# FoundationVision/OmniTokenizer

Measured on NVIDIA H100. Metric: video_frames_per_sec_encode_decode, higher is better.
Workload: dtype f32

## Files before the change

### include/omnitok_b200.h

```cpp
#ifndef OMNITOK_B200_H_
#define OMNITOK_B200_H_

#include <stdint.h>

#ifdef __cplusplus
extern "C" {
#endif

#define OMT_ABI_VERSION 2

#define OMT_OK 0
#define OMT_E_ARG (-1)
#define OMT_E_ARCH (-2)
#define OMT_E_CUDA (-3)
#define OMT_E_UNSUPPORTED (-4)

typedef void* omt_stream_t;

int omt_abi_version(void);
const char* omt_last_error(void);
int omt_device_info(int* sm_count, int* cc_major, int* cc_minor);

#define OMT_EPI_NONE 0
#define OMT_EPI_GEGLU 1
#define OMT_EPI_QKV 2
#define OMT_EPI_QKV_PLANES 3

#define OMT_MATH_FP32 0
#define OMT_MATH_3XTF32 1
#define OMT_MATH_F16X3 3

int omt_linear(const float* A, int lda, int a_seg, int a_seg_stride, int a_seg_off,
               const float* W, const float* W_lo,
               float* C, int ldc, int c_seg, int c_seg_stride, int c_seg_off,
               int M, int N, int K,
               const float* bias, const float* residual, int ldr,
               int epilogue, int math, omt_stream_t stream);

int omt_linear2(const float* A1, const float* A2, int n_split, int lda, const float* W, const float* W_lo,
                float* C, int ldc, int M, int N, int K, int math,
                const float* q_scale, const float* k_scale, const float* rope_cos, const float* rope_sin,
                int qk_cols, int tokens, omt_stream_t stream);

int omt_layernorm(const float* x, int ldx, float* y, int ldy, const float* w, const float* b,
                  int M, int C, float eps, int seg, int seg_stride, int seg_off, omt_stream_t stream);

int omt_patchify_ln(const float* video, float* A, uint16_t* A_hi, uint16_t* A_lo, float* A_rs, const float* ln_w, const float* ln_b,
                    int B, int Cin, int T, int H, int W, int p, int pt, int first, float eps,
                    omt_stream_t stream);

int omt_patchify_ln_u8(const uint8_t* frames, const float* lut, const int32_t* sel, float* A, uint16_t* A_hi, uint16_t* A_lo,
                       float* A_rs, const float* ln_w, const float* ln_b, int B, int Cin, int T, int H, int W, int p, int pt,
                       int first, float eps, omt_stream_t stream);

int omt_u8_norm_select(const uint8_t* frames, int B, long long per_sample, int32_t* sel, omt_stream_t stream);

int omt_unpatchify(const float* P, float* video, int B, int Cin, int T, int H, int W, int p, int pt,
                   int first, omt_stream_t stream);

int omt_unpatchify_u8(const float* P, uint8_t* out, int B, int Cin, int T, int H, int W, int p, int pt,
                      int first, float mul, float add, float lo, float hi, float post, omt_stream_t stream);

int omt_peg(const float* x, float* y, const float* w27, const float* bias, const int32_t* nbr,
            int B, int rows_per_b, int C, omt_stream_t stream);

int omt_peg_volume(const float* x, float* y, const float* w27, const float* bias, int B, int T, int h, int w,
                   int C, int temporal, int causal, omt_stream_t stream);

int omt_qk_prep(float* q, int ldq, float* k, int ldk, const float* q_scale, const float* k_scale,
                const float* rope_cos, const float* rope_sin, int M, int N, int heads,
                omt_stream_t stream);

int omt_attn_spatial(const float* q, int ldq, const float* k, int ldk, const float* v, int ldv,
                     float* o, uint16_t* o_hi, uint16_t* o_lo, int ldo, int n_seq, int N, int heads, float scale,
                     omt_stream_t stream);

int omt_attn_spatial_h(const uint16_t* q_hi, const uint16_t* q_lo, int ldq, const uint16_t* k_hi, const uint16_t* k_lo, int ldk,
                       const uint16_t* v_hi, const uint16_t* v_lo, int ldv, const float* vinv, float qk_plane_scale,
                       float* o, uint16_t* o_hi, uint16_t* o_lo, int ldo, int n_seq, int N, int heads, float scale,
                       omt_stream_t stream);

int omt_attn_window(const float* q, int ldq, const float* k, int ldk, const float* v, int ldv,
                    float* o, uint16_t* o_hi, uint16_t* o_lo, int ldo, const float* bias, int n_frames, int h, int w, int ws, int heads,
                    float scale, omt_stream_t stream);

int omt_attn_temporal(const float* q, int ldq, const float* k, int ldk, const float* v, int ldv,
                      float* o, uint16_t* o_hi, uint16_t* o_lo, int ldo, int B, int T, int N, int heads, float scale, int causal,
                      omt_stream_t stream);

int omt_pre_vq(const float* x, int ldx, const float* Wt, const float* b, float* z, int M, int C, int cd,
               int l2, omt_stream_t stream);

int omt_vq_search(const float* z, const float* E, const float* e2, int M, int n_codes,
                  int64_t* idx, int32_t* counts, omt_stream_t stream);

int omt_vq_fused(const float* x, int ldx, const float* Wt, const float* b, int C, int l2, float* z,
                 const float* E, const float* e2, int M, int n_codes, int64_t* idx, int32_t* counts,
                 omt_stream_t stream);

int omt_post_vq(const int64_t* idx, const float* E, const float* zc, const float* z_st_from,
                float* zq_out, const float* Wt, const float* b, float* X, int M, int C, int cd,
                omt_stream_t stream);

typedef struct omt_linear_h_args {
  const uint16_t* a_hi; const uint16_t* a_lo;
  const float* a_rs; const float* a2_rs;
  float w_scale;
  const uint16_t* a2_hi; const uint16_t* a2_lo;
  int n_split;
  int lda, a_seg, a_seg_stride, a_seg_off;
  const uint16_t* w_hi; const uint16_t* w_lo;
  float* c; int ldc, c_seg, c_seg_stride, c_seg_off;
  uint16_t* u_hi; uint16_t* u_lo; int ldu;
  int M, N, K;
  const float* bias; const float* residual; int ldr;
  int epilogue;
  const float* q_scale; const float* k_scale; const float* rope_cos; const float* rope_sin;
  int qk_cols, tokens;
  float q_plane_scale, k_plane_scale;
  float* vinv;
  float a_rs_uniform, u_scale;
} omt_linear_h_args;

int omt_linear_h(const omt_linear_h_args* args, omt_stream_t stream);

int omt_layernorm_h(const float* x, int ldx, float* y, int ldy, uint16_t* y_hi, uint16_t* y_lo, float* y_rs,
                    uint16_t* x_hi, uint16_t* x_lo, float* x_rs, int lds, const float* w, const float* b,
                    int M, int C, float eps, int seg, int seg_stride, int seg_off, omt_stream_t stream);

int omt_set_option(const char* name, int value);

#ifdef __cplusplus
}
#endif
#endif
```

### omnitokenizer_b200/_cabi.py

```python
from __future__ import annotations

import ctypes
import os
from ctypes import c_char_p, c_float, c_int, c_int64, c_void_p, POINTER

import torch

_LIB_NAME = "libomnitok_b200.so"
_lib = None

EPI_NONE, EPI_GEGLU, EPI_QKV, EPI_QKV_PLANES = 0, 1, 2, 3
MATH_FP32, MATH_3XTF32, MATH_F16X3 = 0, 1, 3
ABI_VERSION = 2


class LinearHArgs(ctypes.Structure):
    _fields_ = [("a_hi", c_void_p), ("a_lo", c_void_p), ("a_rs", c_void_p), ("a2_rs", c_void_p), ("w_scale", c_float),
                ("a2_hi", c_void_p), ("a2_lo", c_void_p), ("n_split", c_int),
                ("lda", c_int), ("a_seg", c_int), ("a_seg_stride", c_int), ("a_seg_off", c_int),
                ("w_hi", c_void_p), ("w_lo", c_void_p),
                ("c", c_void_p), ("ldc", c_int), ("c_seg", c_int), ("c_seg_stride", c_int), ("c_seg_off", c_int),
                ("u_hi", c_void_p), ("u_lo", c_void_p), ("ldu", c_int),
                ("M", c_int), ("N", c_int), ("K", c_int),
                ("bias", c_void_p), ("residual", c_void_p), ("ldr", c_int),
                ("epilogue", c_int),
                ("q_scale", c_void_p), ("k_scale", c_void_p), ("rope_cos", c_void_p), ("rope_sin", c_void_p),
                ("qk_cols", c_int), ("tokens", c_int),
                ("q_plane_scale", c_float), ("k_plane_scale", c_float), ("vinv", c_void_p),
                ("a_rs_uniform", c_float), ("u_scale", c_float)]


SIGNATURES = {
    "omt_abi_version": (c_int, []),
    "omt_last_error": (c_char_p, []),
    "omt_device_info": (c_int, [POINTER(c_int)] * 3),
    "omt_set_option": (c_int, [c_char_p, c_int]),
    "omt_linear": (c_int, [c_void_p, c_int, c_int, c_int, c_int, c_void_p, c_void_p, c_void_p, c_int, c_int, c_int,
                           c_int, c_int, c_int, c_int, c_void_p, c_void_p, c_int, c_int, c_int, c_void_p]),
    "omt_linear2": (c_int, [c_void_p, c_void_p, c_int, c_int, c_void_p, c_void_p, c_void_p, c_int, c_int, c_int, c_int,
                            c_int, c_void_p, c_void_p, c_void_p, c_void_p, c_int, c_int, c_void_p]),
    "omt_linear_h": (c_int, [POINTER(LinearHArgs), c_void_p]),
    "omt_layernorm": (c_int, [c_void_p, c_int, c_void_p, c_int, c_void_p, c_void_p, c_int, c_int, c_float, c_int, c_int,
                              c_int, c_void_p]),
    "omt_layernorm_h": (c_int, [c_void_p, c_int, c_void_p, c_int, c_void_p, c_void_p, c_void_p, c_void_p, c_void_p, c_void_p,
                                c_int, c_void_p, c_void_p, c_int, c_int, c_float, c_int, c_int, c_int, c_void_p]),
    "omt_patchify_ln": (c_int, [c_void_p, c_void_p, c_void_p, c_void_p, c_void_p, c_void_p, c_void_p] + [c_int] * 8 + [c_float, c_void_p]),
    "omt_patchify_ln_u8": (c_int, [c_void_p] * 9 + [c_int] * 8 + [c_float, c_void_p]),
    "omt_u8_norm_select": (c_int, [c_void_p, c_int, c_int64, c_void_p, c_void_p]),
    "omt_unpatchify": (c_int, [c_void_p, c_void_p] + [c_int] * 8 + [c_void_p]),
    "omt_unpatchify_u8": (c_int, [c_void_p, c_void_p] + [c_int] * 8 + [c_float] * 5 + [c_void_p]),
    "omt_peg": (c_int, [c_void_p, c_void_p, c_void_p, c_void_p, c_void_p, c_int, c_int, c_int, c_void_p]),
    "omt_peg_volume": (c_int, [c_void_p, c_void_p, c_void_p, c_void_p] + [c_int] * 7 + [c_void_p]),
    "omt_qk_prep": (c_int, [c_void_p, c_int, c_void_p, c_int, c_void_p, c_void_p, c_void_p, c_void_p, c_int, c_int,
                            c_int, c_void_p]),
    "omt_attn_spatial": (c_int, [c_void_p, c_int, c_void_p, c_int, c_void_p, c_int, c_void_p, c_void_p, c_void_p, c_int,
                                 c_int, c_int, c_int, c_float, c_void_p]),
    "omt_attn_spatial_h": (c_int, [c_void_p, c_void_p, c_int, c_void_p, c_void_p, c_int, c_void_p, c_void_p, c_int, c_void_p,
                                   c_float, c_void_p, c_void_p, c_void_p, c_int, c_int, c_int, c_int, c_float, c_void_p]),
    "omt_attn_window": (c_int, [c_void_p, c_int, c_void_p, c_int, c_void_p, c_int, c_void_p, c_void_p, c_void_p, c_int,
                                c_void_p, c_int, c_int, c_int, c_int, c_int, c_float, c_void_p]),
    "omt_attn_temporal": (c_int, [c_void_p, c_int, c_void_p, c_int, c_void_p, c_int, c_void_p, c_void_p, c_void_p, c_int,
                                  c_int, c_int, c_int, c_int, c_float, c_int, c_void_p]),
    "omt_pre_vq": (c_int, [c_void_p, c_int, c_void_p, c_void_p, c_void_p, c_int, c_int, c_int, c_int, c_void_p]),
    "omt_vq_search": (c_int, [c_void_p, c_void_p, c_void_p, c_int, c_int, c_void_p, c_void_p, c_void_p]),
    "omt_vq_fused": (c_int, [c_void_p, c_int, c_void_p, c_void_p, c_int, c_int, c_void_p, c_void_p, c_void_p, c_int, c_int,
                             c_void_p, c_void_p, c_void_p]),
    "omt_post_vq": (c_int, [c_void_p] * 8 + [c_int, c_int, c_int, c_void_p]),
}


def lib_path() -> str:
    return os.environ.get("OMT_LIB") or os.path.join(os.path.dirname(os.path.abspath(__file__)), _LIB_NAME)


def load():
    global _lib
    if _lib is not None:
        return _lib
    path = lib_path()
    if not os.path.exists(path):
        raise RuntimeError(
            f"{path} not found: the CUDA extension is not built. Run `python -c 'import __graft_entry__ as g; "
            f"g.build()'` (or `make -C omnitokenizer_b200/csrc`). There is no CPU fallback.")
    lib = ctypes.CDLL(path)
    for name, (res, args) in SIGNATURES.items():
        fn = getattr(lib, name)
        fn.restype = res
        fn.argtypes = args
    if lib.omt_abi_version() != ABI_VERSION:
        raise RuntimeError("libomnitok_b200.so ABI version mismatch")
    _lib = lib
    return lib


def _ptr(t):
    if t is None:
        return None
    if isinstance(t, int):
        return t
    return t.data_ptr()


def _stream():
    return torch.cuda.current_stream().cuda_stream


KERNELS_PER_CALL = {"omt_u8_norm_select": 2}
launch_count = 0


def call(name: str, *args):
    global launch_count
    lib = load()
    launch_count += KERNELS_PER_CALL.get(name, 1)
    conv = [_ptr(a) if (a is None or isinstance(a, torch.Tensor)) else a for a in args]
    rc = getattr(lib, name)(*conv, _stream())
    if rc != 0:
        raise RuntimeError(f"{name} failed ({rc}): {lib.omt_last_error().decode()}")


def linear_h(**kw):
    global launch_count
    lib = load()
    a = LinearHArgs()
    for k, v in kw.items():
        setattr(a, k, _ptr(v) if (v is None or isinstance(v, torch.Tensor)) else v)
    launch_count += 1
    rc = lib.omt_linear_h(ctypes.byref(a), _stream())
    if rc != 0:
        raise RuntimeError(f"omt_linear_h failed ({rc}): {lib.omt_last_error().decode()}")


DEFAULT_OPTIONS = {"attn_kernel": 3, "peg_kernel": 4, "f16_bn": 0, "attn_f16_ctas": 2}


def set_option(name: str, value: int):
    lib = load()
    rc = lib.omt_set_option(name.encode(), int(value))
    if rc != 0:
        raise RuntimeError(f"omt_set_option({name}) failed: {lib.omt_last_error().decode()}")


def device_info():
    lib = load()
    a, b, c = c_int(), c_int(), c_int()
    rc = lib.omt_device_info(ctypes.byref(a), ctypes.byref(b), ctypes.byref(c))
    if rc != 0:
        raise RuntimeError(lib.omt_last_error().decode())
    return a.value, b.value, c.value
```

### omnitokenizer_b200/csrc/attention_f16.cu

```cuda
#include "omt_common.cuh"
#include "tc_ptx.cuh"
#include <cuda.h>

namespace omt {
int g_attn_f16_ctas = 2;
namespace af16 {
using namespace omt::ptx;

constexpr int QT = 128, KT = 64, D = 64;
constexpr int TILE = KT * D * 2;
constexpr int STAGES = 4;
constexpr int OFF_Q = 0;
constexpr int OFF_KV = 4 * TILE;
constexpr int OFF_VI = OFF_KV + STAGES * 4 * TILE;
constexpr int OFF_CTRL = OFF_VI + STAGES * KT * 4;
constexpr int SMEM = OFF_CTRL + 128 + 1024;
constexpr int THREADS = 384;
constexpr uint32_t KV_BYTES = 4 * TILE + KT * 4;
constexpr int PRODUCER_REGS = 40, CONSUMER_REGS = 232;

struct Args {
  const float* vinv;
  long long rows;
  float* o; uint16_t* o_hi; uint16_t* o_lo; int ldo;
  int N, heads, items;
  float scale_log2;
};

__global__ void __launch_bounds__(THREADS, 1)
attn_f16_kernel(const __grid_constant__ CUtensorMap tmQh, const __grid_constant__ CUtensorMap tmQl,
                const __grid_constant__ CUtensorMap tmKh, const __grid_constant__ CUtensorMap tmKl,
                const __grid_constant__ CUtensorMap tmVh, const __grid_constant__ CUtensorMap tmVl, const Args a) {
  extern __shared__ uint8_t smem_raw[];
  uint8_t* smem = smem_raw + ((1024u - (smem_u32(smem_raw) & 1023u)) & 1023u);
  uint64_t* bars = reinterpret_cast<uint64_t*>(smem + OFF_CTRL);
  uint64_t& q_full = bars[0];
  uint64_t& q_empty = bars[1];
  uint64_t* full = bars + 2;
  uint64_t* empty = full + STAGES;
  float* vmax = reinterpret_cast<float*>(bars + 2 + 2 * STAGES);

  const int tid = threadIdx.x, warp = tid >> 5, lane = tid & 31;
  const int ntiles = a.N / KT, nqt = a.N / QT;

  if (tid == 0) {
    prefetch_map(&tmQh); prefetch_map(&tmQl); prefetch_map(&tmKh); prefetch_map(&tmKl); prefetch_map(&tmVh); prefetch_map(&tmVl);
    mbar_init(&q_full, 1);
    mbar_init(&q_empty, 256);
    for (int s = 0; s < STAGES; ++s) { mbar_init(&full[s], 1); mbar_init(&empty[s], 2); }
    fence_barrier_init();
  }
  __syncthreads();
  pdl_sync();

  auto decode = [&](int item, int& row_q0, int& row_k0, int& col0, int& head) {
    const int qt = item % nqt, hs = item / nqt, seq = hs / a.heads;
    head = hs % a.heads;
    row_k0 = seq * a.N;
    row_q0 = row_k0 + qt * QT;
    col0 = head * D;
  };

  if (warp < 4) {
    setmaxnreg_dec<PRODUCER_REGS>();
    if (warp == 0) {
      uint32_t it = 0, c = 0;
      for (int item = blockIdx.x; item < a.items; item += gridDim.x, ++c) {
        int row_q0, row_k0, col0, head;
        decode(item, row_q0, row_k0, col0, head);
        const float* vinv_h = a.vinv + (size_t)head * a.rows + row_k0;
        float vmx = 0.f;
        for (int i = 4 * lane; i < a.N; i += 128) {
          const float4 v = __ldg(reinterpret_cast<const float4*>(vinv_h + i));
          vmx = fmaxf(vmx, fmaxf(fmaxf(v.x, v.y), fmaxf(v.z, v.w)));
        }
        vmx = warp_max(vmx);
        mbar_wait(&q_empty, (c & 1) ^ 1);
        if (lane == 0) {
          *vmax = vmx;
          mbar_expect_tx(&q_full, 4 * TILE);
          for (int w = 0; w < 2; ++w) {
            tma_load_2d(&tmQh, &q_full, smem + OFF_Q + w * TILE, col0, row_q0 + w * 64);
            tma_load_2d(&tmQl, &q_full, smem + OFF_Q + (2 + w) * TILE, col0, row_q0 + w * 64);
          }
        }
        for (int j = 0; j < ntiles; ++j, ++it) {
          const int s = it % STAGES;
          mbar_wait(&empty[s], ((it / STAGES) & 1) ^ 1);
          if (lane == 0) {
            uint8_t* sp = smem + OFF_KV + s * 4 * TILE;
            const int kr = row_k0 + j * KT;
            mbar_expect_tx(&full[s], KV_BYTES);
            tma_load_2d(&tmKh, &full[s], sp, col0, kr);
            tma_load_2d(&tmKl, &full[s], sp + TILE, col0, kr);
            tma_load_2d(&tmVh, &full[s], sp + 2 * TILE, col0, kr);
            tma_load_2d(&tmVl, &full[s], sp + 3 * TILE, col0, kr);
            bulk_load(smem + OFF_VI + s * KT * 4, vinv_h + j * KT, KT * 4, &full[s]);
          }
        }
      }
    }
  } else {
    setmaxnreg_inc<CONSUMER_REGS>();
    const int wg = (warp >> 2) - 1, qd = lane & 3;
    const int rl0 = (warp & 3) * 16 + (lane >> 2);
    const uint32_t sb = smem_u32(smem);
    auto release = [&](uint32_t t) {
      if ((tid & 127) == 0) mbar_arrive(&empty[t % STAGES]);
    };
    float sv[32];
#pragma unroll
    for (int i = 0; i < 32; ++i) sv[i] = 0.f;
    uint32_t it = 0, c = 0;
    for (int item = blockIdx.x; item < a.items; item += gridDim.x, ++c) {
      int row_q0, row_k0, col0, head;
      decode(item, row_q0, row_k0, col0, head);
      mbar_wait(&q_full, c & 1);
      float p_scale, p_inv;
      row_scale(*vmax, p_scale, p_inv);
      uint32_t qh[16], ql[16];
#pragma unroll
      for (int kk = 0; kk < 4; ++kk)
#pragma unroll
        for (int e = 0; e < 2; ++e)
#pragma unroll
          for (int h = 0; h < 2; ++h) {
            const int r = rl0 + 8 * h;
            const uint8_t* p = smem + OFF_Q + wg * TILE + r * 128 + (((2 * kk + e) ^ (r & 7)) << 4) + qd * 4;
            qh[4 * kk + 2 * e + h] = *reinterpret_cast<const uint32_t*>(p);
            ql[4 * kk + 2 * e + h] = *reinterpret_cast<const uint32_t*>(p + 2 * TILE);
          }
      mbar_arrive(&q_empty);

      float o_acc[32];
#pragma unroll
      for (int i = 0; i < 32; ++i) o_acc[i] = 0.f;
      float m_run[2] = {-INFINITY, -INFINITY}, l_run[2] = {0.f, 0.f};
      uint32_t p_a[2][16], p_b[2][16];
      float alpha[2];

      auto wait_full = [&](uint32_t t) { mbar_wait(&full[t % STAGES], (t / STAGES) & 1); };
      auto issue_s = [&](uint32_t t) {
        const uint32_t kv = sb + OFF_KV + (t % STAGES) * 4 * TILE;
        const uint64_t dk_hi = desc_sw128(kv), dk_lo = desc_sw128(kv + TILE);
#pragma unroll
        for (int kk = 0; kk < 4; ++kk) {
          const uint64_t adv = (uint64_t)(kk * 2);
          wgmma_f16_n64_ra<0>(sv, ql + 4 * kk, dk_hi + adv, kk != 0);
          wgmma_f16_n64_ra<0>(sv, qh + 4 * kk, dk_lo + adv, 1);
          wgmma_f16_n64_ra<0>(sv, qh + 4 * kk, dk_hi + adv, 1);
        }
      };
      auto issue_pv = [&](const uint32_t (&p)[2][16], uint32_t t) {
        const uint32_t vh = sb + OFF_KV + (t % STAGES) * 4 * TILE + 2 * TILE, vl = vh + TILE;
#pragma unroll
        for (int kk = 0; kk < 4; ++kk) {
          const uint64_t dvh = desc_sw128(vh + kk * 2048), dvl = desc_sw128(vl + kk * 2048);
          wgmma_f16_n64_ra<1>(o_acc, p[1] + 4 * kk, dvh, 1);
          wgmma_f16_n64_ra<1>(o_acc, p[0] + 4 * kk, dvl, 1);
          wgmma_f16_n64_ra<1>(o_acc, p[0] + 4 * kk, dvh, 1);
        }
      };
      auto softmax = [&](uint32_t (&p)[2][16], uint32_t t) {
        float nm[2];
#pragma unroll
        for (int h = 0; h < 2; ++h) {
          float mx = -INFINITY;
#pragma unroll
          for (int jj = 0; jj < 8; ++jj) mx = fmaxf(mx, fmaxf(sv[4 * jj + 2 * h], sv[4 * jj + 2 * h + 1]));
          mx = fmaxf(mx, __shfl_xor_sync(0xffffffffu, mx, 1));
          mx = fmaxf(mx, __shfl_xor_sync(0xffffffffu, mx, 2));
          const float m_new = fmaxf(m_run[h], mx);
          alpha[h] = ex2_fast((m_run[h] - m_new) * a.scale_log2);
          m_run[h] = m_new;
          nm[h] = -m_new;
        }
        const float* vi = reinterpret_cast<const float*>(smem + OFF_VI + (t % STAGES) * KT * 4);
        float ps[2] = {0.f, 0.f};
#pragma unroll
        for (int jj = 0; jj < 8; ++jj) {
          const float2 w = *reinterpret_cast<const float2*>(vi + 8 * jj + 2 * qd);
#pragma unroll
          for (int h = 0; h < 2; ++h) {
            const float e0 = ex2_fast((sv[4 * jj + 2 * h] + nm[h]) * a.scale_log2);
            const float e1 = ex2_fast((sv[4 * jj + 2 * h + 1] + nm[h]) * a.scale_log2);
            ps[h] += e0 + e1;
            const int wd = 4 * (jj >> 1) + 2 * (jj & 1) + h;
            split2u(e0 * (w.x * p_scale), e1 * (w.y * p_scale), p[0][wd], p[1][wd]);
          }
        }
#pragma unroll
        for (int h = 0; h < 2; ++h) l_run[h] = fmaf(l_run[h], alpha[h], ps[h]);
      };
      auto rescale = [&]() {
#pragma unroll
        for (int h = 0; h < 2; ++h)
#pragma unroll
          for (int jj = 0; jj < 8; ++jj) { o_acc[4 * jj + 2 * h] *= alpha[h]; o_acc[4 * jj + 2 * h + 1] *= alpha[h]; }
      };
      auto step = [&](const uint32_t (&p)[2][16], uint32_t (&pn)[2][16], int j, bool next) {
        const uint32_t t = it + j;
        if (next) wait_full(t + 1);
        reg_fence(sv);
        reg_fence(o_acc);
        wg_fence();
        if (next) {
          issue_s(t + 1);
          wg_commit();
        }
        issue_pv(p, t);
        wg_commit();
        if (next) {
          wg_wait<1>();
          reg_fence(sv);
          softmax(pn, t + 1);
        }
        wg_wait<0>();
        reg_fence(o_acc);
        release(t);
        if (next) rescale();
      };

      wait_full(it);
      reg_fence(sv);
      wg_fence();
      issue_s(it);
      wg_commit();
      wg_wait<0>();
      reg_fence(sv);
      softmax(p_a, it);
      rescale();
      int j = 0;
      for (; j + 2 < ntiles; j += 2) {
        step(p_a, p_b, j, true);
        step(p_b, p_a, j + 1, true);
      }
      step(p_a, p_b, j, true);
      step(p_b, p_a, j + 1, false);
      it += ntiles;

#pragma unroll
      for (int h = 0; h < 2; ++h) {
        float l = l_run[h];
        l += __shfl_xor_sync(0xffffffffu, l, 1);
        l += __shfl_xor_sync(0xffffffffu, l, 2);
        const float inv = p_inv / l;
        const size_t ooff = (size_t)(row_q0 + wg * 64 + rl0 + 8 * h) * a.ldo + col0 + 2 * qd;
#pragma unroll
        for (int jj = 0; jj < 8; ++jj) {
          const float2 ov = make_float2(o_acc[4 * jj + 2 * h] * inv, o_acc[4 * jj + 2 * h + 1] * inv);
          if (a.o_hi != nullptr) store_split2(a.o_hi, a.o_lo, ooff + 8 * jj, ov);
          else *reinterpret_cast<float2*>(a.o + ooff + 8 * jj) = ov;
        }
      }
    }
  }
}

typedef CUresult (*EncodeTiledFn)(CUtensorMap*, CUtensorMapDataType, cuuint32_t, void*, const cuuint64_t*,
                                  const cuuint64_t*, const cuuint32_t*, const cuuint32_t*, CUtensorMapInterleave,
                                  CUtensorMapSwizzle, CUtensorMapL2promotion, CUtensorMapFloatOOBfill);

static int encode2d(CUtensorMap* m, const uint16_t* base, int cols, long long rows, int ld) {
  static EncodeTiledFn fn = nullptr;
  if (fn == nullptr) {
    void* p = nullptr;
    cudaDriverEntryPointQueryResult qres;
    if (cudaGetDriverEntryPoint("cuTensorMapEncodeTiled", &p, cudaEnableDefault, &qres) == cudaSuccess &&
        qres == cudaDriverEntryPointSuccess)
      fn = reinterpret_cast<EncodeTiledFn>(p);
  }
  if (fn == nullptr) { set_error("cuTensorMapEncodeTiled entry point not found"); return OMT_E_CUDA; }
  cuuint64_t dims[2] = {(cuuint64_t)cols, (cuuint64_t)rows};
  cuuint64_t strides[1] = {(cuuint64_t)ld * 2};
  cuuint32_t box[2] = {64, (cuuint32_t)KT};
  cuuint32_t estr[2] = {1, 1};
  CUresult r = fn(m, CU_TENSOR_MAP_DATA_TYPE_FLOAT16, 2, const_cast<uint16_t*>(base), dims, strides, box, estr,
                  CU_TENSOR_MAP_INTERLEAVE_NONE, CU_TENSOR_MAP_SWIZZLE_128B, CU_TENSOR_MAP_L2_PROMOTION_L2_256B,
                  CU_TENSOR_MAP_FLOAT_OOB_FILL_NONE);
  if (r != CUDA_SUCCESS) { set_error("cuTensorMapEncodeTiled failed (%d)", (int)r); return OMT_E_CUDA; }
  return OMT_OK;
}

}
}

using namespace omt;

extern "C" int omt_attn_spatial_h(const uint16_t* q_hi, const uint16_t* q_lo, int ldq, const uint16_t* k_hi,
                                  const uint16_t* k_lo, int ldk, const uint16_t* v_hi, const uint16_t* v_lo, int ldv,
                                  const float* vinv, float qk_plane_scale, float* o, uint16_t* o_hi, uint16_t* o_lo, int ldo,
                                  int n_seq, int N, int heads, float scale, omt_stream_t stream) {
  using namespace af16;
  OMT_ENTER();
  OMT_REQUIRE(q_hi && q_lo && k_hi && k_lo && v_hi && v_lo && vinv && (o || o_hi) && ((o_hi == nullptr) == (o_lo == nullptr)),
              "omt_attn_spatial_h: null pointer");
  OMT_REQUIRE(N > 0 && N % QT == 0, "omt_attn_spatial_h: N=%d must be a multiple of 128", N);
  OMT_REQUIRE(ldq % 8 == 0 && ldk % 8 == 0 && ldv % 8 == 0 && ldo % 4 == 0, "omt_attn_spatial_h: bad leading dims");
  OMT_REQUIRE(((uintptr_t)q_hi | (uintptr_t)q_lo | (uintptr_t)k_hi | (uintptr_t)k_lo | (uintptr_t)v_hi | (uintptr_t)v_lo | (uintptr_t)vinv |
               (uintptr_t)o | (uintptr_t)o_hi | (uintptr_t)o_lo) % 16 == 0, "omt_attn_spatial_h: pointers must be 16-byte aligned");
  OMT_REQUIRE(heads > 0 && heads <= 65535 && n_seq <= 65535 && qk_plane_scale > 0.f, "omt_attn_spatial_h: bad arguments");
  if (n_seq == 0) return OMT_OK;
  const long long rows = (long long)n_seq * N;
  const long long items = rows / QT * heads;
  OMT_REQUIRE(rows < (1LL << 31) && items < (1LL << 31), "omt_attn_spatial_h: n_seq * N = %lld rows is too many", rows);
  CUtensorMap tmQh, tmQl, tmKh, tmKl, tmVh, tmVl;
  int rc;
  if ((rc = encode2d(&tmQh, q_hi, heads * D, rows, ldq))) return rc;
  if ((rc = encode2d(&tmQl, q_lo, heads * D, rows, ldq))) return rc;
  if ((rc = encode2d(&tmKh, k_hi, heads * D, rows, ldk))) return rc;
  if ((rc = encode2d(&tmKl, k_lo, heads * D, rows, ldk))) return rc;
  if ((rc = encode2d(&tmVh, v_hi, heads * D, rows, ldv))) return rc;
  if ((rc = encode2d(&tmVl, v_lo, heads * D, rows, ldv))) return rc;
  static int resident[64];
  int dev = 0;
  OMT_CUDA(cudaGetDevice(&dev));
  OMT_REQUIRE(dev >= 0 && dev < 64, "omt_attn_spatial_h: device ordinal %d out of range", dev);
  if (resident[dev] == 0) {
    OMT_CUDA(cudaFuncSetAttribute(attn_f16_kernel, cudaFuncAttributeMaxDynamicSharedMemorySize, SMEM));
    int per_sm = 0, sms = 0;
    OMT_CUDA(cudaOccupancyMaxActiveBlocksPerMultiprocessor(&per_sm, attn_f16_kernel, THREADS, SMEM));
    OMT_CUDA(cudaDeviceGetAttribute(&sms, cudaDevAttrMultiProcessorCount, dev));
    OMT_REQUIRE(per_sm > 0, "omt_attn_spatial_h: no CTA fits on an SM of device %d", dev);
    resident[dev] = per_sm * sms;
  }
  Args a{vinv, rows, o, o_hi, o_lo, ldo, N, heads, (int)items, scale * 1.4426950408889634f / qk_plane_scale};
  const dim3 grid(items < resident[dev] ? (int)items : resident[dev]);
  OMT_CUDA(launch_k(attn_f16_kernel, grid, dim3(THREADS), SMEM, (cudaStream_t)stream, tmQh, tmQl, tmKh, tmKl, tmVh, tmVl, a));
  OMT_LAUNCH_CHECK();
  return OMT_OK;
}
```

### omnitokenizer_b200/csrc/attention_fp32.cu

```cuda
#include "omt_common.cuh"

namespace omt {

constexpr int AQ = 64;
constexpr int AK = 64;
constexpr int AD = 64;

__device__ __forceinline__ int sw(int r, int c) { return r * 64 + ((c ^ ((r >> 2) & 7)) << 2); }

struct AttnArgs {
  const float* q; int ldq;
  const float* k; int ldk;
  const float* v; int ldv;
  float* o; int ldo;
  uint16_t* o_hi; uint16_t* o_lo;
  const float* bias;
  int N;
  int h, w, ws;
  float scale;
};

template <bool WINDOW>
__device__ __forceinline__ long long token_row(const AttnArgs& a, int seq, int i) {
  if (!WINDOW) return (long long)seq * a.N + i;
  const int nwx = a.w / a.ws;
  const int nW = (a.h / a.ws) * nwx;
  const int frame = seq / nW, win = seq % nW;
  const int wy = win / nwx, wx = win % nwx;
  const int sy = i / a.ws, sx = i % a.ws;
  return (long long)frame * a.N + (wy * a.ws + sy) * a.w + wx * a.ws + sx;
}

template <bool WINDOW>
__global__ void __launch_bounds__(256, 2) attn_flash_kernel(const AttnArgs a) {
  pdl_sync();
  extern __shared__ __align__(16) float smem[];
  float* Qs = smem;
  float* Ks = smem + 4096;
  float* Vs = smem + 8192;
  float* Ps = smem + 12288;
  const int tid = threadIdx.x;
  const int tx = tid & 15, ty = tid >> 4;
  const int qt = WINDOW ? 0 : blockIdx.x, head = blockIdx.y;
  const int seq = WINDOW ? blockIdx.x : blockIdx.z;
  const int seq_len = WINDOW ? 64 : a.N;
  const int lc = tid & 15, lr = tid >> 4;

#pragma unroll
  for (int it = 0; it < 4; ++it) {
    const int r = lr + it * 16;
    const long long row = token_row<WINDOW>(a, seq, qt * AQ + r);
    float4 v = *reinterpret_cast<const float4*>(a.q + row * a.ldq + head * AD + lc * 4);
    v.x *= a.scale; v.y *= a.scale; v.z *= a.scale; v.w *= a.scale;
    *reinterpret_cast<float4*>(Qs + sw(r, lc)) = v;
  }

  float o[4][4];
  float mrow[4], lrow[4];
#pragma unroll
  for (int i = 0; i < 4; ++i) {
    mrow[i] = -INFINITY; lrow[i] = 0.f;
#pragma unroll
    for (int j = 0; j < 4; ++j) o[i][j] = 0.f;
  }

  float4 pk[4], pv[4];
  auto prefetch = [&](int kc) {
#pragma unroll
    for (int it = 0; it < 4; ++it) {
      const int r = lr + it * 16;
      const long long row = token_row<WINDOW>(a, seq, kc * AK + r);
      pk[it] = *reinterpret_cast<const float4*>(a.k + row * a.ldk + head * AD + lc * 4);
      pv[it] = *reinterpret_cast<const float4*>(a.v + row * a.ldv + head * AD + lc * 4);
    }
  };
  const int nkc = seq_len / AK;
  prefetch(0);
  for (int kc = 0; kc < nkc; ++kc) {
    __syncthreads();
#pragma unroll
    for (int it = 0; it < 4; ++it) {
      const int r = lr + it * 16;
      *reinterpret_cast<float4*>(Ks + sw(r, lc)) = pk[it];
      *reinterpret_cast<float4*>(Vs + r * 64 + lc * 4) = pv[it];
    }
    __syncthreads();
    if (kc + 1 < nkc) prefetch(kc + 1);

    float s[4][4];
#pragma unroll
    for (int i = 0; i < 4; ++i)
#pragma unroll
      for (int j = 0; j < 4; ++j) s[i][j] = 0.f;
#pragma unroll 4
    for (int c = 0; c < 16; ++c) {
      float4 qf[4], kf[4];
#pragma unroll
      for (int i = 0; i < 4; ++i) qf[i] = *reinterpret_cast<const float4*>(Qs + sw(ty * 4 + i, c));
#pragma unroll
      for (int j = 0; j < 4; ++j) kf[j] = *reinterpret_cast<const float4*>(Ks + sw(tx * 4 + j, c));
#pragma unroll
      for (int i = 0; i < 4; ++i)
#pragma unroll
        for (int j = 0; j < 4; ++j) {
          s[i][j] = fmaf(qf[i].x, kf[j].x, s[i][j]);
          s[i][j] = fmaf(qf[i].y, kf[j].y, s[i][j]);
          s[i][j] = fmaf(qf[i].z, kf[j].z, s[i][j]);
          s[i][j] = fmaf(qf[i].w, kf[j].w, s[i][j]);
        }
    }
    if (WINDOW) {
#pragma unroll
      for (int i = 0; i < 4; ++i) {
        const float4 b = *reinterpret_cast<const float4*>(a.bias + ((size_t)head * 64 + ty * 4 + i) * 64 + tx * 4);
        s[i][0] += b.x; s[i][1] += b.y; s[i][2] += b.z; s[i][3] += b.w;
      }
    }
#pragma unroll
    for (int i = 0; i < 4; ++i) {
      float mx = fmaxf(fmaxf(s[i][0], s[i][1]), fmaxf(s[i][2], s[i][3]));
#pragma unroll
      for (int off = 8; off > 0; off >>= 1) mx = fmaxf(mx, __shfl_xor_sync(0xffffffffu, mx, off));
      const float mnew = fmaxf(mrow[i], mx);
      const float corr = expf(mrow[i] - mnew);
      float ps = 0.f;
#pragma unroll
      for (int j = 0; j < 4; ++j) { s[i][j] = expf(s[i][j] - mnew); ps += s[i][j]; }
#pragma unroll
      for (int off = 8; off > 0; off >>= 1) ps += __shfl_xor_sync(0xffffffffu, ps, off);
      lrow[i] = lrow[i] * corr + ps;
      mrow[i] = mnew;
#pragma unroll
      for (int j = 0; j < 4; ++j) o[i][j] *= corr;
      *reinterpret_cast<float4*>(Ps + sw(ty * 4 + i, tx)) = make_float4(s[i][0], s[i][1], s[i][2], s[i][3]);
    }
    __syncthreads();
#pragma unroll 4
    for (int jc = 0; jc < 16; ++jc) {
      float4 pf[4];
#pragma unroll
      for (int i = 0; i < 4; ++i) pf[i] = *reinterpret_cast<const float4*>(Ps + sw(ty * 4 + i, jc));
#pragma unroll
      for (int jj = 0; jj < 4; ++jj) {
        const float4 vf = *reinterpret_cast<const float4*>(Vs + (jc * 4 + jj) * 64 + tx * 4);
#pragma unroll
        for (int i = 0; i < 4; ++i) {
          const float p = (jj == 0) ? pf[i].x : (jj == 1) ? pf[i].y : (jj == 2) ? pf[i].z : pf[i].w;
          o[i][0] = fmaf(p, vf.x, o[i][0]);
          o[i][1] = fmaf(p, vf.y, o[i][1]);
          o[i][2] = fmaf(p, vf.z, o[i][2]);
          o[i][3] = fmaf(p, vf.w, o[i][3]);
        }
      }
    }
  }
#pragma unroll
  for (int i = 0; i < 4; ++i) {
    const long long row = token_row<WINDOW>(a, seq, qt * AQ + ty * 4 + i);
    const float inv = 1.0f / lrow[i];
    const float4 ov = make_float4(o[i][0] * inv, o[i][1] * inv, o[i][2] * inv, o[i][3] * inv);
    if (a.o_hi != nullptr) store_split4(a.o_hi, a.o_lo, (size_t)(row * a.ldo + head * AD + tx * 4), ov);
    else *reinterpret_cast<float4*>(a.o + row * a.ldo + head * AD + tx * 4) = ov;
  }
}

template <int T>
__global__ void __launch_bounds__(256) attn_temporal_kernel(const float* __restrict__ q, int ldq,
                                                            const float* __restrict__ k, int ldk,
                                                            const float* __restrict__ v, int ldv,
                                                            float* __restrict__ o, uint16_t* __restrict__ o_hi,
                                                            uint16_t* __restrict__ o_lo, int ldo, int B,
                                                            int N, int heads, float scale, int causal) {
  pdl_sync();
  const int lane = threadIdx.x & 31;
  const long long wid = (long long)blockIdx.x * (blockDim.x >> 5) + (threadIdx.x >> 5);
  const long long total = (long long)B * N * heads;
  if (wid >= total) return;
  const int head = (int)(wid % heads);
  const long long bn = wid / heads;
  const int n = (int)(bn % N);
  const int b = (int)(bn / N);
  const size_t col = (size_t)head * 64 + 2 * lane;
  float2 kr[T], vr[T], qr[T];
#pragma unroll
  for (int t = 0; t < T; ++t) {
    const size_t row = ((size_t)b * T + t) * N + n;
    kr[t] = *reinterpret_cast<const float2*>(k + row * ldk + col);
    vr[t] = *reinterpret_cast<const float2*>(v + row * ldv + col);
    qr[t] = *reinterpret_cast<const float2*>(q + row * ldq + col);
  }
#pragma unroll
  for (int i = 0; i < T; ++i) {
    const size_t row = ((size_t)b * T + i) * N + n;
    const float2 qv = qr[i];
    float s[T];
#pragma unroll
    for (int j = 0; j < T; ++j) s[j] = qv.x * kr[j].x + qv.y * kr[j].y;
#pragma unroll
    for (int off = 16; off > 0; off >>= 1)
#pragma unroll
      for (int j = 0; j < T; ++j) s[j] += __shfl_xor_sync(0xffffffffu, s[j], off);
    float mx = -INFINITY;
#pragma unroll
    for (int j = 0; j < T; ++j) {
      s[j] *= scale;
      if (!causal || j <= i) mx = fmaxf(mx, s[j]);
    }
    float den = 0.f, ox = 0.f, oy = 0.f;
#pragma unroll
    for (int j = 0; j < T; ++j) {
      if (!causal || j <= i) {
        const float p = expf(s[j] - mx);
        den += p;
        ox = fmaf(p, vr[j].x, ox);
        oy = fmaf(p, vr[j].y, oy);
      }
    }
    const float2 ov = make_float2(ox / den, oy / den);
    if (o_hi != nullptr) store_split2(o_hi, o_lo, row * ldo + col, ov);
    else *reinterpret_cast<float2*>(o + row * ldo + col) = ov;
  }
}

template <int T>
static int launch_temporal(const float* q, int ldq, const float* k, int ldk, const float* v, int ldv,
                           float* o, uint16_t* o_hi, uint16_t* o_lo, int ldo, int B, int N, int heads, float scale, int causal,
                           cudaStream_t st) {
  const long long warps = (long long)B * N * heads;
  const unsigned blocks = (unsigned)((warps + 7) / 8);
  OMT_CUDA(launch_k(attn_temporal_kernel<T>, dim3(blocks), dim3(256), 0, st, q, ldq, k, ldk, v, ldv, o, o_hi, o_lo, ldo, B, N, heads, scale, causal));
  OMT_LAUNCH_CHECK();
  return OMT_OK;
}

int launch_attn_tc3(const float* q, int ldq, const float* k, int ldk, const float* v, int ldv, float* o, uint16_t* o_hi,
                    uint16_t* o_lo, int ldo, int n_seq, int N, int heads, float scale, cudaStream_t st);
int g_attn_kernel = 3;

static int set_flash_smem() {
  static bool done[64];
  int dev = 0;
  cudaGetDevice(&dev);
  if (dev >= 0 && dev < 64 && !done[dev]) {
    OMT_CUDA(cudaFuncSetAttribute(attn_flash_kernel<false>, cudaFuncAttributeMaxDynamicSharedMemorySize, 65536));
    OMT_CUDA(cudaFuncSetAttribute(attn_flash_kernel<true>, cudaFuncAttributeMaxDynamicSharedMemorySize, 65536));
    done[dev] = true;
  }
  return OMT_OK;
}

}

using namespace omt;

static int check_attn_ptrs(const char* who, const float* q, int ldq, const float* k, int ldk, const float* v,
                           int ldv, float* o, uint16_t* o_hi, uint16_t* o_lo, int ldo) {
  OMT_REQUIRE(q && k && v && (o || o_hi) && ((o_hi == nullptr) == (o_lo == nullptr)), "%s: null pointer", who);
  OMT_REQUIRE(((uintptr_t)o_hi | (uintptr_t)o_lo) % 8 == 0, "%s: output planes must be 8-byte aligned", who);
  OMT_REQUIRE(ldq % 4 == 0 && ldk % 4 == 0 && ldv % 4 == 0 && ldo % 4 == 0, "%s: leading dims must be multiples of 4", who);
  OMT_REQUIRE(((uintptr_t)q | (uintptr_t)k | (uintptr_t)v | (uintptr_t)o) % 16 == 0, "%s: pointers must be 16-byte aligned", who);
  return OMT_OK;
}

extern "C" int omt_attn_spatial(const float* q, int ldq, const float* k, int ldk, const float* v, int ldv,
                                float* o, uint16_t* o_hi, uint16_t* o_lo, int ldo, int n_seq, int N, int heads, float scale,
                                omt_stream_t stream) {
  OMT_ENTER();
  int rc = check_attn_ptrs("omt_attn_spatial", q, ldq, k, ldk, v, ldv, o, o_hi, o_lo, ldo);
  if (rc) return rc;
  OMT_REQUIRE(N > 0 && N % 64 == 0, "omt_attn_spatial: N=%d must be a multiple of 64", N);
  OMT_REQUIRE(heads > 0 && heads <= 65535 && n_seq <= 65535, "omt_attn_spatial: grid too large");
  if (n_seq == 0) return OMT_OK;
  if (g_attn_kernel == 3 && N % 128 == 0)
    return launch_attn_tc3(q, ldq, k, ldk, v, ldv, o, o_hi, o_lo, ldo, n_seq, N, heads, scale, (cudaStream_t)stream);
  rc = set_flash_smem();
  if (rc) return rc;
  AttnArgs a{q, ldq, k, ldk, v, ldv, o, ldo, o_hi, o_lo, nullptr, N, 0, 0, 0, scale};
  dim3 grid(N / AQ, heads, n_seq);
  OMT_CUDA(launch_k(attn_flash_kernel<false>, grid, dim3(256), 65536, (cudaStream_t)stream, a));
  OMT_LAUNCH_CHECK();
  return OMT_OK;
}

extern "C" int omt_attn_window(const float* q, int ldq, const float* k, int ldk, const float* v, int ldv,
                               float* o, uint16_t* o_hi, uint16_t* o_lo, int ldo, const float* bias, int n_frames, int h,
                               int w, int ws, int heads, float scale, omt_stream_t stream) {
  OMT_ENTER();
  int rc = check_attn_ptrs("omt_attn_window", q, ldq, k, ldk, v, ldv, o, o_hi, o_lo, ldo);
  if (rc) return rc;
  OMT_REQUIRE(bias != nullptr, "omt_attn_window: null bias");
  OMT_REQUIRE(ws * ws == 64, "omt_attn_window: window %dx%d unsupported (8x8 only)", ws, ws);
  OMT_REQUIRE(h % ws == 0 && w % ws == 0, "omt_attn_window: grid %dx%d not divisible by the window", h, w);
  const long long n_seq = (long long)n_frames * (h / ws) * (w / ws);
  OMT_REQUIRE(n_seq <= 0x7fffffffLL / 64, "omt_attn_window: too many windows");
  if (n_seq == 0) return OMT_OK;
  rc = set_flash_smem();
  if (rc) return rc;
  AttnArgs a{q, ldq, k, ldk, v, ldv, o, ldo, o_hi, o_lo, bias, h * w, h, w, ws, scale};
  dim3 grid((unsigned)n_seq, heads, 1);
  OMT_CUDA(launch_k(attn_flash_kernel<true>, grid, dim3(256), 65536, (cudaStream_t)stream, a));
  OMT_LAUNCH_CHECK();
  return OMT_OK;
}

extern "C" int omt_attn_temporal(const float* q, int ldq, const float* k, int ldk, const float* v, int ldv,
                                 float* o, uint16_t* o_hi, uint16_t* o_lo, int ldo, int B, int T, int N, int heads,
                                 float scale, int causal, omt_stream_t stream) {
  OMT_ENTER();
  int rc = check_attn_ptrs("omt_attn_temporal", q, ldq, k, ldk, v, ldv, o, o_hi, o_lo, ldo);
  if (rc) return rc;
  OMT_REQUIRE(T >= 1 && T <= 17, "omt_attn_temporal: T'=%d unsupported (1..17)", T);
  if ((long long)B * N == 0) return OMT_OK;
  cudaStream_t st = (cudaStream_t)stream;
#define OMT_T_CASE(t) case t: return launch_temporal<t>(q, ldq, k, ldk, v, ldv, o, o_hi, o_lo, ldo, B, N, heads, scale, causal, st);
  switch (T) {
    OMT_T_CASE(1) OMT_T_CASE(2) OMT_T_CASE(3) OMT_T_CASE(4) OMT_T_CASE(5) OMT_T_CASE(6) OMT_T_CASE(7)
    OMT_T_CASE(8) OMT_T_CASE(9) OMT_T_CASE(10) OMT_T_CASE(11) OMT_T_CASE(12) OMT_T_CASE(13) OMT_T_CASE(14)
    OMT_T_CASE(15) OMT_T_CASE(16) OMT_T_CASE(17)
  }
#undef OMT_T_CASE
  return OMT_E_ARG;
}
```

### omnitokenizer_b200/csrc/gemm_wgmma.cuh

```cuda
#pragma once
#include "omt_common.cuh"
#include "tc_ptx.cuh"
#include <cuda.h>

namespace omt {
namespace wgg {
using namespace omt::ptx;

constexpr int BM = 128, BN = 128;
constexpr int THREADS = 384;
constexpr int ORDER_BAR = 3;
constexpr int STAGE_BYTES = 4 * 16384;
constexpr int STAGES = 3;
constexpr int SMEM = STAGES * STAGE_BYTES + 1024;
constexpr int PRODUCER_REGS = 40, CONSUMER_REGS = 232;

struct Args {
  int M, N, K;
  int num_m_blk, n_split;
  int a_seg, a_seg_stride, a_seg_off;
  const float* a_rs; const float* a2_rs;
  float a_rs_uniform;
  float w_scale;
  float u_scale;
  float* c; int ldc;
  int c_seg, c_seg_stride, c_seg_off;
  const float* bias;
  const float* residual; int ldr;
  uint16_t* u_hi; uint16_t* u_lo; int ldu;
  const float* rope_cos; const float* rope_sin; const float* q_scale; const float* k_scale;
  int qk_cols; int tokens;
  float q_ps, k_ps;
  float* vinv;
};

template <bool TF32, int NACC, int EPI>
__device__ __forceinline__ void epilogue(const Args& g, const float (&acc)[BN / 2], const float (&crs)[NACC == 2 ? BN / 2 : 1],
                                         int m0, int n0, bool second, int half, int warp, int lane) {
  const int qd = lane & 3;
  int mrow[2];
  mrow[0] = m0 + half * 64 + (warp & 3) * 16 + (lane >> 2);
  mrow[1] = mrow[0] + 8;
  float v[2][BN / 4];
#pragma unroll
  for (int h = 0; h < 2; ++h) {
    float os = 1.f;
    if (!TF32 && NACC == 1) {
      const float* rs = second ? g.a2_rs : g.a_rs;
      const int m = mrow[h];
      os = g.w_scale * (rs == nullptr ? g.a_rs_uniform : (m < g.M ? __ldg(rs + map_row(m, g.a_seg, g.a_seg_stride, g.a_seg_off)) : 1.0f));
    }
#pragma unroll
    for (int j = 0; j < BN / 8; ++j)
#pragma unroll
      for (int e = 0; e < 2; ++e) {
        const int i = 4 * j + 2 * h + e;
        float x = acc[i];
        if constexpr (!TF32 && NACC == 2) x = fmaf(crs[i], 1.0f / F16X3_LO_SCALE, x);
        if (!TF32 && NACC == 1) x = x * os;
        v[h][2 * j + e] = x;
      }
  }

  if constexpr (EPI == OMT_EPI_QKV || EPI == OMT_EPI_QKV_PLANES) {
#pragma unroll
    for (int hd = 0; hd < BN / 64; ++hd) {
      const int nh = n0 + hd * 64;
      if (nh >= g.N) break;
#pragma unroll
      for (int h = 0; h < 2; ++h) {
        const int m = mrow[h];
        float* x = &v[h][hd * 16];
        if (nh < g.qk_cols) {
          if (g.rope_cos != nullptr) {
            const int pos = (m < g.M ? m : 0) % g.tokens;
#pragma unroll
            for (int j = 0; j < 8; ++j) {
              const int p = 4 * j + qd;
              const float cc = __ldg(g.rope_cos + (size_t)pos * 32 + p), ss = __ldg(g.rope_sin + (size_t)pos * 32 + p);
              const float a = x[2 * j], b = x[2 * j + 1];
              x[2 * j] = a * cc - b * ss;
              x[2 * j + 1] = a * ss + b * cc;
            }
          }
          float sq = 0.f;
#pragma unroll
          for (int i = 0; i < 16; ++i) sq = fmaf(x[i], x[i], sq);
          sq += __shfl_xor_sync(0xffffffffu, sq, 1);
          sq += __shfl_xor_sync(0xffffffffu, sq, 2);
          const float inv = 1.0f / fmaxf(sqrtf(sq), 1e-12f);
          const float* scv = (nh < g.qk_cols / 2) ? g.q_scale : g.k_scale;
#pragma unroll
          for (int j = 0; j < 8; ++j) {
            const float2 s2 = __ldg(reinterpret_cast<const float2*>(scv + 8 * j + 2 * qd));
            x[2 * j] = x[2 * j] * inv * s2.x;
            x[2 * j + 1] = x[2 * j + 1] * inv * s2.y;
          }
        }
        if constexpr (EPI == OMT_EPI_QKV) {
          if (m < g.M) {
            float* crow = g.c + map_row(m, g.c_seg, g.c_seg_stride, g.c_seg_off) * g.ldc + nh + 2 * qd;
#pragma unroll
            for (int j = 0; j < 8; ++j) *reinterpret_cast<float2*>(crow + 8 * j) = make_float2(x[2 * j], x[2 * j + 1]);
          }
        } else {
          float sc = nh < g.qk_cols / 2 ? g.q_ps : g.k_ps;
          if (nh >= g.qk_cols) {
            float mx = 0.f;
#pragma unroll
            for (int i = 0; i < 16; ++i) mx = fmaxf(mx, fabsf(x[i]));
            mx = fmaxf(mx, __shfl_xor_sync(0xffffffffu, mx, 1));
            mx = fmaxf(mx, __shfl_xor_sync(0xffffffffu, mx, 2));
            float inv;
            row_scale(mx, sc, inv);
            if (m < g.M && qd == 0) g.vinv[(size_t)((nh - g.qk_cols) >> 6) * g.M + m] = inv;
          }
          if (m < g.M) {
            const size_t off = (size_t)m * g.ldu + nh + 2 * qd;
#pragma unroll
            for (int j = 0; j < 8; ++j) {
              uint32_t hw, lw;
              split2u(x[2 * j] * sc, x[2 * j + 1] * sc, hw, lw);
              *reinterpret_cast<uint32_t*>(g.u_hi + off + 8 * j) = hw;
              *reinterpret_cast<uint32_t*>(g.u_lo + off + 8 * j) = lw;
            }
          }
        }
      }
    }
  } else if constexpr (EPI == OMT_EPI_GEGLU) {
#pragma unroll
    for (int h = 0; h < 2; ++h) {
      const int m = mrow[h];
      const long long prow = map_row(m < g.M ? m : 0, g.c_seg, g.c_seg_stride, g.c_seg_off);
#pragma unroll
      for (int j = 0; j < BN / 8; ++j) {
        const int n = n0 + 8 * j + 2 * qd;
        float val = v[h][2 * j], gate = v[h][2 * j + 1];
        if (g.bias != nullptr && n < g.N) { val += __ldg(g.bias + n); gate += __ldg(g.bias + n + 1); }
        const float o = gelu_erf(gate) * val;
        const float o1 = __shfl_xor_sync(0xffffffffu, o, 1);
        if ((qd & 1) == 0 && m < g.M && n < g.N) {
          if (TF32) {
            *reinterpret_cast<float2*>(g.c + prow * g.ldc + (n >> 1)) = make_float2(o, o1);
          } else {
            uint32_t hw, lw;
            if (g.u_scale > 0.f) split2u(o * g.u_scale, o1 * g.u_scale, hw, lw);
            else split2(o, o1, hw, lw);
            const size_t off = (size_t)prow * g.ldu + (n >> 1);
            *reinterpret_cast<uint32_t*>(g.u_hi + off) = hw;
            *reinterpret_cast<uint32_t*>(g.u_lo + off) = lw;
          }
        }
      }
    }
  } else {
#pragma unroll
    for (int h = 0; h < 2; ++h) {
      const int m = mrow[h];
      if (m < g.M) {
        const long long prow = map_row(m, g.c_seg, g.c_seg_stride, g.c_seg_off);
#pragma unroll
        for (int j = 0; j < BN / 8; ++j) {
          const int n = n0 + 8 * j + 2 * qd;
          if (n < g.N) {
            float2 o = make_float2(v[h][2 * j], v[h][2 * j + 1]);
            if (g.bias != nullptr) {
              const float2 bb = __ldg(reinterpret_cast<const float2*>(g.bias + n));
              o.x += bb.x; o.y += bb.y;
            }
            if (g.residual != nullptr) {
              const float2 r = *reinterpret_cast<const float2*>(g.residual + prow * g.ldr + n);
              o.x += r.x; o.y += r.y;
            }
            *reinterpret_cast<float2*>(g.c + prow * g.ldc + n) = o;
          }
        }
      }
    }
  }
}

template <bool TF32, int NACC, int EPI>
__global__ void __launch_bounds__(THREADS, 1)
gemm_wgmma_kernel(const __grid_constant__ CUtensorMap tmA, const __grid_constant__ CUtensorMap tmAl,
                  const __grid_constant__ CUtensorMap tmA2, const __grid_constant__ CUtensorMap tmA2l,
                  const __grid_constant__ CUtensorMap tmWh, const __grid_constant__ CUtensorMap tmWl, const Args g) {
  constexpr int BK = TF32 ? 32 : 64;
  constexpr bool PINGPONG = !TF32 && NACC == 1;
  constexpr int HALVES = PINGPONG ? 2 : 1;
  constexpr int A_BYTES = BM * 128, W_BYTES = BN * 128;
  constexpr uint32_t TX_BYTES = TF32 ? A_BYTES + 2 * W_BYTES : 2 * A_BYTES + 2 * W_BYTES;
  extern __shared__ uint8_t smem_raw[];
  uint8_t* smem = smem_raw + ((1024u - (smem_u32(smem_raw) & 1023u)) & 1023u);
  __shared__ __align__(8) uint64_t full[STAGES], empty[STAGES];

  const int tid = threadIdx.x, warp = tid >> 5, lane = tid & 31;
  const int num_kb = g.K / BK;
  const int num_n_blk = (g.N + BN - 1) / BN;
  const int num_tiles = g.num_m_blk * num_n_blk;

  if (tid == 0) {
    prefetch_map(&tmA); prefetch_map(&tmA2); prefetch_map(&tmWh); prefetch_map(&tmWl);
    if (!TF32) { prefetch_map(&tmAl); prefetch_map(&tmA2l); }
    for (int s = 0; s < STAGES; ++s) {
      mbar_init(&full[s], 1);
      mbar_init(&empty[s], PINGPONG ? 1 : 2);
    }
    fence_barrier_init();
  }
  __syncthreads();
  pdl_sync();

  auto tile_origin = [&](int t, int& m0, int& n0) { m0 = (t / num_n_blk) * BM; n0 = (t % num_n_blk) * BN; };

  if (warp < 4) {
    setmaxnreg_dec<PRODUCER_REGS>();
    if (tid == 0) {
      uint32_t it = 0;
      for (int tile = blockIdx.x; tile < num_tiles; tile += gridDim.x) {
        int m0, n0;
        tile_origin(tile, m0, n0);
        const bool second = n0 >= g.n_split;
        int c1[2], c2[2];
#pragma unroll
        for (int hf = 0; hf < 2; ++hf) {
          const int r = m0 + hf * 64;
          if (g.a_seg > 0) { c1[hf] = r % g.a_seg; c2[hf] = r / g.a_seg; }
          else { c1[hf] = r; c2[hf] = 0; }
        }
        const CUtensorMap* mah = second ? &tmA2 : &tmA;
        const CUtensorMap* mal = second ? &tmA2l : &tmAl;
        for (int kb = 0; kb < num_kb; ++kb, ++it) {
          const int s = it % STAGES;
          uint8_t* sp = smem + (size_t)s * STAGE_BYTES;
          mbar_wait(&empty[s], ((it / STAGES) & 1) ^ 1);
          mbar_expect_tx(&full[s], TX_BYTES);
          tma_load_3d(mah, &full[s], sp, kb * BK, c1[0], c2[0]);
          tma_load_3d(mah, &full[s], sp + A_BYTES / 2, kb * BK, c1[1], c2[1]);
          if (!TF32) {
            tma_load_3d(mal, &full[s], sp + A_BYTES, kb * BK, c1[0], c2[0]);
            tma_load_3d(mal, &full[s], sp + A_BYTES + A_BYTES / 2, kb * BK, c1[1], c2[1]);
          }
          tma_load_2d(&tmWh, &full[s], sp + 2 * A_BYTES, kb * BK, n0);
          tma_load_2d(&tmWl, &full[s], sp + 2 * A_BYTES + W_BYTES, kb * BK, n0);
        }
      }
    }
  } else {
    setmaxnreg_inc<CONSUMER_REGS>();
    const int wg = (warp >> 2) - 1;
    auto release = [&](uint32_t i) {
      if ((tid & 127) == 0) mbar_arrive(&empty[i % STAGES]);
    };
    uint32_t it = PINGPONG ? wg * num_kb : 0;
    for (int tile = blockIdx.x + (PINGPONG ? wg : 0) * gridDim.x; tile < num_tiles; tile += (PINGPONG ? 2 : 1) * gridDim.x) {
      int m0, n0;
      tile_origin(tile, m0, n0);
      const bool second = n0 >= g.n_split;
      float acc[HALVES][BN / 2], crs[NACC == 2 ? BN / 2 : 1];
#pragma unroll
      for (int h = 0; h < HALVES; ++h)
#pragma unroll
        for (int i = 0; i < BN / 2; ++i) acc[h][i] = 0.f;
#pragma unroll
      for (int i = 0; i < (NACC == 2 ? BN / 2 : 1); ++i) crs[i] = 0.f;
      if (PINGPONG && tile != (int)blockIdx.x) named_bar_sync(ORDER_BAR + wg, 256);

      for (int kb = 0; kb < num_kb; ++kb, ++it) {
        const int s = it % STAGES;
        uint8_t* sp = smem + (size_t)s * STAGE_BYTES;
        mbar_wait(&full[s], (it / STAGES) & 1);
        if (TF32) {
          float4* a = reinterpret_cast<float4*>(sp + wg * (A_BYTES / 2));
          float4* alo = reinterpret_cast<float4*>(sp + A_BYTES + wg * (A_BYTES / 2));
          const int t = tid & 127;
#pragma unroll
          for (int i = 0; i < 4; ++i) {
            const int idx = t + i * 128;
            const float4 v = a[idx];
            float4 hi, lo;
            hi.x = tf32_rn(v.x); hi.y = tf32_rn(v.y); hi.z = tf32_rn(v.z); hi.w = tf32_rn(v.w);
            lo.x = v.x - hi.x; lo.y = v.y - hi.y; lo.z = v.z - hi.z; lo.w = v.w - hi.w;
            a[idx] = hi;
            alo[idx] = lo;
          }
          fence_async_smem();
          wg_bar(1 + wg);
        }
        const uint32_t sa = smem_u32(sp);
        const uint64_t d_whi = desc_sw128(sa + 2 * A_BYTES), d_wlo = desc_sw128(sa + 2 * A_BYTES + W_BYTES);
        wg_fence();
#pragma unroll
        for (int k = 0; k < 4; ++k) {
          const uint64_t adv = (uint64_t)(k * 2);
#pragma unroll
          for (int h = 0; h < HALVES; ++h) {
            const int r = PINGPONG ? h : wg;
            const uint64_t d_ahi = desc_sw128(sa + r * (A_BYTES / 2)), d_alo = desc_sw128(sa + A_BYTES + r * (A_BYTES / 2));
            if constexpr (TF32) {
              wgmma_tf32_n128(acc[h], d_alo + adv, d_whi + adv, 1);
              wgmma_tf32_n128(acc[h], d_ahi + adv, d_wlo + adv, 1);
              wgmma_tf32_n128(acc[h], d_ahi + adv, d_whi + adv, 1);
            } else if constexpr (NACC == 2) {
              wgmma_f16_n128(crs, d_alo + adv, d_whi + adv, 1);
              wgmma_f16_n128(crs, d_ahi + adv, d_wlo + adv, 1);
              wgmma_f16_n128(acc[h], d_ahi + adv, d_whi + adv, 1);
            } else {
              wgmma_f16_n128(acc[h], d_alo + adv, d_whi + adv, 1);
              wgmma_f16_n128(acc[h], d_ahi + adv, d_wlo + adv, 1);
              wgmma_f16_n128(acc[h], d_ahi + adv, d_whi + adv, 1);
            }
          }
        }
        wg_commit();
        wg_wait<1>();
        if (kb > 0) release(it - 1);
      }
      if (PINGPONG && tile + (int)gridDim.x < num_tiles) named_bar_arrive(ORDER_BAR + (wg ^ 1), 256);
      wg_wait<0>();
      release(it - 1);
      if (PINGPONG) it += num_kb;
#pragma unroll
      for (int h = 0; h < HALVES; ++h)
        epilogue<TF32, NACC, EPI>(g, acc[h], crs, m0, n0, second, PINGPONG ? h : wg, warp, lane);
    }
  }
}

typedef CUresult (*EncodeTiledFn)(CUtensorMap*, CUtensorMapDataType, cuuint32_t, void*, const cuuint64_t*,
                                  const cuuint64_t*, const cuuint32_t*, const cuuint32_t*, CUtensorMapInterleave,
                                  CUtensorMapSwizzle, CUtensorMapL2promotion, CUtensorMapFloatOOBfill);

static inline int encode_map(CUtensorMap* m, CUtensorMapDataType dt, const void* base, int rank, const cuuint64_t* dims,
                             const cuuint64_t* strides, const cuuint32_t* box) {
  static EncodeTiledFn fn = nullptr;
  if (fn == nullptr) {
    void* p = nullptr;
    cudaDriverEntryPointQueryResult qres;
    if (cudaGetDriverEntryPoint("cuTensorMapEncodeTiled", &p, cudaEnableDefault, &qres) == cudaSuccess &&
        qres == cudaDriverEntryPointSuccess)
      fn = reinterpret_cast<EncodeTiledFn>(p);
  }
  if (fn == nullptr) { set_error("cuTensorMapEncodeTiled entry point not found"); return OMT_E_CUDA; }
  cuuint32_t estr[5] = {1, 1, 1, 1, 1};
  CUresult r = fn(m, dt, (cuuint32_t)rank, const_cast<void*>(base), dims, strides, box, estr, CU_TENSOR_MAP_INTERLEAVE_NONE,
                  CU_TENSOR_MAP_SWIZZLE_128B, CU_TENSOR_MAP_L2_PROMOTION_L2_256B, CU_TENSOR_MAP_FLOAT_OOB_FILL_NONE);
  if (r != CUDA_SUCCESS) { set_error("cuTensorMapEncodeTiled failed (%d)", (int)r); return OMT_E_CUDA; }
  return OMT_OK;
}

static inline int row_map(CUtensorMap* m, CUtensorMapDataType dt, int esize, const void* ptr, int ld, int rows, int cols,
                          int seg, int seg_stride, int seg_off) {
  const int s = seg > 0 ? seg : rows;
  const int nseg = seg > 0 ? rows / seg : 1;
  const long long sstride = seg > 0 ? seg_stride : rows;
  cuuint64_t dims[3] = {(cuuint64_t)cols, (cuuint64_t)s, (cuuint64_t)nseg};
  cuuint64_t strides[2] = {(cuuint64_t)ld * esize, (cuuint64_t)sstride * ld * esize};
  cuuint32_t box[3] = {(cuuint32_t)(128 / esize), 64, 1};
  const uint8_t* base = static_cast<const uint8_t*>(ptr) + (size_t)(seg > 0 ? seg_off : 0) * ld * esize;
  return encode_map(m, dt, base, 3, dims, strides, box);
}

static inline int w_map(CUtensorMap* m, CUtensorMapDataType dt, int esize, const void* ptr, int n_pad, int K) {
  cuuint64_t dims[2] = {(cuuint64_t)K, (cuuint64_t)n_pad};
  cuuint64_t strides[1] = {(cuuint64_t)K * esize};
  cuuint32_t box[2] = {(cuuint32_t)(128 / esize), (cuuint32_t)BN};
  return encode_map(m, dt, ptr, 2, dims, strides, box);
}

template <bool TF32, int NACC, int EPI>
static int launch(const CUtensorMap* maps, const Args& g, cudaStream_t st) {
  auto kern = gemm_wgmma_kernel<TF32, NACC, EPI>;
  static int resident[64];
  int dev = 0;
  OMT_CUDA(cudaGetDevice(&dev));
  OMT_REQUIRE(dev >= 0 && dev < 64, "wgmma GEMM: device ordinal %d out of range", dev);
  if (resident[dev] == 0) {
    OMT_CUDA(cudaFuncSetAttribute(kern, cudaFuncAttributeMaxDynamicSharedMemorySize, SMEM));
    int per_sm = 0, sms = 0;
    OMT_CUDA(cudaOccupancyMaxActiveBlocksPerMultiprocessor(&per_sm, kern, THREADS, SMEM));
    OMT_CUDA(cudaDeviceGetAttribute(&sms, cudaDevAttrMultiProcessorCount, dev));
    OMT_REQUIRE(per_sm > 0, "wgmma GEMM: no CTA fits on an SM of device %d", dev);
    resident[dev] = per_sm * sms;
  }
  const int tiles = g.num_m_blk * ((g.N + BN - 1) / BN);
  const dim3 grid(tiles < resident[dev] ? tiles : resident[dev]);
  OMT_CUDA(launch_k(kern, grid, dim3(THREADS), SMEM, st, maps[0], maps[1], maps[2], maps[3], maps[4], maps[5], g));
  OMT_LAUNCH_CHECK();
  return OMT_OK;
}

}
}
```

### omnitokenizer_b200/csrc/omt_common.cuh

```cuda
#pragma once
#include <cuda_runtime.h>
#include <stdint.h>
#include <stdio.h>
#include <stdarg.h>
#include "../../include/omnitok_b200.h"

namespace omt {

void set_error(const char* fmt, ...);
int check_device();
int sm_count();

#define OMT_REQUIRE(cond, ...)                  \
  do {                                          \
    if (!(cond)) {                              \
      omt::set_error(__VA_ARGS__);              \
      return OMT_E_ARG;                         \
    }                                           \
  } while (0)

#define OMT_CUDA(call)                                                            \
  do {                                                                            \
    cudaError_t e__ = (call);                                                     \
    if (e__ != cudaSuccess) {                                                     \
      omt::set_error("%s failed: %s (%s:%d)", #call, cudaGetErrorString(e__),     \
                     __FILE__, __LINE__);                                         \
      return OMT_E_CUDA;                                                          \
    }                                                                             \
  } while (0)

#define OMT_ENTER()                      \
  do {                                   \
    int rc__ = omt::check_device();      \
    if (rc__ != OMT_OK) return rc__;     \
  } while (0)

#define OMT_LAUNCH_CHECK() OMT_CUDA(cudaGetLastError())

__device__ __forceinline__ void pdl_sync() {
  asm volatile("griddepcontrol.wait;" ::: "memory");
  asm volatile("griddepcontrol.launch_dependents;" ::: "memory");
}
extern int g_pdl;

template <typename... KArgs, typename... Args>
inline cudaError_t launch_k(void (*kernel)(KArgs...), dim3 grid, dim3 block, size_t smem, cudaStream_t st, Args... args) {
  cudaLaunchConfig_t cfg = {};
  cfg.gridDim = grid; cfg.blockDim = block; cfg.dynamicSmemBytes = smem; cfg.stream = st;
  cudaLaunchAttribute at[1];
  at[0].id = cudaLaunchAttributeProgrammaticStreamSerialization;
  at[0].val.programmaticStreamSerializationAllowed = 1;
  cfg.attrs = at; cfg.numAttrs = g_pdl ? 1 : 0;
  return cudaLaunchKernelEx(&cfg, kernel, KArgs(args)...);
}

__device__ __forceinline__ float warp_sum(float v) {
#pragma unroll
  for (int o = 16; o > 0; o >>= 1) v += __shfl_xor_sync(0xffffffffu, v, o);
  return v;
}
__device__ __forceinline__ float warp_max(float v) {
#pragma unroll
  for (int o = 16; o > 0; o >>= 1) v = fmaxf(v, __shfl_xor_sync(0xffffffffu, v, o));
  return v;
}

constexpr float F16X3_LO_SCALE = 2048.0f;
__device__ __forceinline__ uint32_t pack_f16x2_sat(float a, float b) {
  uint32_t r;
  asm("cvt.rn.satfinite.f16x2.f32 %0, %1, %2;" : "=r"(r) : "f"(b), "f"(a));
  return r;
}
__device__ __forceinline__ float2 unpack_f16x2(uint32_t h) {
  float2 f;
  asm("{\n\t.reg .b16 l, u;\n\tmov.b32 {l, u}, %2;\n\tcvt.f32.f16 %0, l;\n\tcvt.f32.f16 %1, u;\n\t}" : "=f"(f.x), "=f"(f.y) : "r"(h));
  return f;
}
__device__ __forceinline__ void split2(float a, float b, uint32_t& hi2, uint32_t& lo2) {
  hi2 = pack_f16x2_sat(a, b);
  const float2 h = unpack_f16x2(hi2);
  lo2 = pack_f16x2_sat((a - h.x) * F16X3_LO_SCALE, (b - h.y) * F16X3_LO_SCALE);
}
__device__ __forceinline__ void store_split4(uint16_t* hi, uint16_t* lo, size_t off, float4 v) {
  uint2 h, l;
  split2(v.x, v.y, h.x, l.x);
  split2(v.z, v.w, h.y, l.y);
  *reinterpret_cast<uint2*>(hi + off) = h;
  *reinterpret_cast<uint2*>(lo + off) = l;
}
__device__ __forceinline__ void store_split2(uint16_t* hi, uint16_t* lo, size_t off, float2 v) {
  uint32_t h, l;
  split2(v.x, v.y, h, l);
  *reinterpret_cast<uint32_t*>(hi + off) = h;
  *reinterpret_cast<uint32_t*>(lo + off) = l;
}

__device__ __forceinline__ void row_scale(float mx, float& scale, float& inv) {
  uint32_t eb = (__float_as_uint(mx) >> 23) & 0xffu;
  eb = eb < 15u ? 15u : (eb > 254u ? 254u : eb);
  scale = __uint_as_float((268u - eb) << 23);
  inv = __uint_as_float((eb - 14u) << 23);
}
__device__ __forceinline__ void split2u(float a, float b, uint32_t& hi2, uint32_t& lo2) {
  hi2 = pack_f16x2_sat(a, b);
  const float2 h = unpack_f16x2(hi2);
  lo2 = pack_f16x2_sat(a - h.x, b - h.y);
}
__device__ __forceinline__ void store_split4u(uint16_t* hi, uint16_t* lo, size_t off, float4 v, float scale) {
  uint2 h, l;
  split2u(v.x * scale, v.y * scale, h.x, l.x);
  split2u(v.z * scale, v.w * scale, h.y, l.y);
  *reinterpret_cast<uint2*>(hi + off) = h;
  *reinterpret_cast<uint2*>(lo + off) = l;
}
__device__ __forceinline__ float2 ffma2(float2 a, float2 b, float2 c) { return make_float2(fmaf(a.x, b.x, c.x), fmaf(a.y, b.y, c.y)); }
__device__ __forceinline__ float2 fmul2(float2 a, float2 b) { return make_float2(__fmul_rn(a.x, b.x), __fmul_rn(a.y, b.y)); }
__device__ __forceinline__ float2 fadd2(float2 a, float2 b) { return make_float2(__fadd_rn(a.x, b.x), __fadd_rn(a.y, b.y)); }
__device__ __forceinline__ float ex2_fast(float x) {
  float y;
  asm("ex2.approx.ftz.f32 %0, %1;" : "=f"(y) : "f"(x));
  return y;
}
__device__ __forceinline__ void split2u_pk(float2 v, uint32_t& hi2, uint32_t& lo2) {
  hi2 = pack_f16x2_sat(v.x, v.y);
  const float2 d = ffma2(unpack_f16x2(hi2), make_float2(-1.f, -1.f), v);
  lo2 = pack_f16x2_sat(d.x, d.y);
}
__device__ __forceinline__ void store_split8u(uint16_t* hi, uint16_t* lo, size_t off, float4 a, float4 b, float scale) {
  uint4 h, l;
  split2u(a.x * scale, a.y * scale, h.x, l.x);
  split2u(a.z * scale, a.w * scale, h.y, l.y);
  split2u(b.x * scale, b.y * scale, h.z, l.z);
  split2u(b.z * scale, b.w * scale, h.w, l.w);
  *reinterpret_cast<uint4*>(hi + off) = h;
  *reinterpret_cast<uint4*>(lo + off) = l;
}
__device__ __forceinline__ float max4abs(float4 v) { return fmaxf(fmaxf(fabsf(v.x), fabsf(v.y)), fmaxf(fabsf(v.z), fabsf(v.w))); }

__device__ __forceinline__ float gelu_erf(float x) {
  return 0.5f * x * (1.0f + erff(x * 0.70710678118654752440f));
}

__host__ __device__ __forceinline__ long long map_row(int r, int seg, int seg_stride, int seg_off) {
  if (seg <= 0) return r;
  return (long long)(r / seg) * seg_stride + seg_off + (r % seg);
}

struct GemmArgs {
  const float* A; int lda; int a_seg, a_seg_stride, a_seg_off;
  const float* W;
  float* C; int ldc; int c_seg, c_seg_stride, c_seg_off;
  int M, N, K;
  const float* bias; const float* residual; int ldr;
  const float* A2; int n_split;
  const float* rope_cos; const float* rope_sin; const float* q_scale; const float* k_scale;
  int qk_cols; int tokens;
};

}
```

### omnitokenizer_b200/engine.py

```python
from __future__ import annotations

import math
import os
from typing import Dict, Optional, Tuple

import torch

from . import _cabi
from . import layout as L

MATH_MODES = {"fp32": _cabi.MATH_FP32, "3xtf32": _cabi.MATH_3XTF32, "f16x3": _cabi.MATH_F16X3}
DEFAULT_MATH = "f16x3"
VQ_MAX_CODES = 41856


def default_math() -> str:
    return os.environ.get("OMT_MATH", DEFAULT_MATH).lower()


class Planes:

    def __init__(self, device, M: int, ld: int, row_scaled: bool = False):
        self.buf = torch.empty(2, M, ld, device=device, dtype=torch.int16)
        self.hi, self.lo, self.ld = self.buf[0], self.buf[1], ld
        self.rs = torch.empty(M, device=device, dtype=torch.float32) if row_scaled else None


class PackedLinear:

    def __init__(self, weight: torch.Tensor, bias: Optional[torch.Tensor], device, math: int,
                 k_pad: Optional[int] = None, geglu: Optional[Tuple[int, int]] = None, row_scaled: bool = False):
        w = weight.detach().to(device=device, dtype=torch.float32)
        if geglu is not None:
            inner, ku = geglu
            w = L.pack_geglu(w, inner, ku)
        self.n = w.shape[0]
        if k_pad is not None:
            w = L.pad_cols(w, k_pad)
        self.k = w.shape[1]
        w = L.pad_rows(w, 256 if math == _cabi.MATH_F16X3 else 128)
        if math == _cabi.MATH_3XTF32:
            hi = L.tf32_round(w)
            self.w, self.w_lo = hi, (w - hi).contiguous()
        elif math == _cabi.MATH_F16X3 and row_scaled:
            self.w, self.w_lo, self.w_scale = L.split_f16_rs(w)
        elif math == _cabi.MATH_F16X3:
            self.w, self.w_lo = L.split_f16(w)
        else:
            self.w, self.w_lo = w, None
        self.bias = None if bias is None else bias.detach().to(device=device, dtype=torch.float32).contiguous()
        self.math = math
        self.row_scaled = row_scaled and math == _cabi.MATH_F16X3


class Workspace:
    def __init__(self, device, M: int, C: int, ku: int, kmax: int, cd: int, planes: bool):
        f = dict(device=device, dtype=torch.float32)
        self.M = M
        self.buf0 = torch.empty(M, C, **f)
        self.buf1 = torch.empty(M, C, **f)
        self.X, self.Y = self.buf0, self.buf1
        self.QKV = torch.empty(M, 3 * C, **f)
        self.P = torch.empty(M, kmax, **f)
        if planes:
            self.XNp, self.XSp = Planes(device, M, C, True), Planes(device, M, C, True)
            self.Op, self.Up = Planes(device, M, C), Planes(device, M, ku)
            self.Pp = Planes(device, M, kmax, True)
            self.QKVp = Planes(device, M, 3 * C)
            self.vinv = torch.empty(C // 64, M, device=device, dtype=torch.float32)
        else:
            self.XN = torch.empty(M, C, **f)
            self.O = torch.empty(M, C, **f)
            self.U = torch.empty(M, ku, **f)
        self.z = torch.empty(M, cd, **f)
        self.idx = torch.empty(M, device=device, dtype=torch.int64)
        self.counts = torch.zeros(8192, device=device, dtype=torch.int32)
        self.x_in = None
        self.u8_in, self.u8_sel = None, None
        self.video_u8 = None
        self.idx_in = torch.empty(M, device=device, dtype=torch.int64)
        self.zc_in = torch.empty(M, cd, **f)
        self.zq = torch.empty(M, cd, **f)
        self.video = None
        self.graphs = {}

    def reset(self):
        self.X, self.Y = self.buf0, self.buf1


class Engine:
    def __init__(self, model, device: torch.device, math: Optional[str] = None):
        _cabi.load()
        _cabi.set_option("pdl", int(os.environ.get("OMT_PDL", "0")))
        for env, opt in (("OMT_PEG_KERNEL", "peg_kernel"),
                         ("OMT_ATTN_CTAS", "attn_f16_ctas"),
                         ("OMT_F16_BN", "f16_bn")):
            _cabi.set_option(opt, int(os.environ.get(env) or _cabi.DEFAULT_OPTIONS[opt]))
        self.device = device
        self.math_name = (math or default_math()).lower()
        if self.math_name not in MATH_MODES:
            raise ValueError(f"unknown OMT_MATH mode {self.math_name!r}; choose from {sorted(MATH_MODES)}")
        self.math = MATH_MODES[self.math_name]
        a = model.args
        self.C = a.embedding_dim
        self.heads, self.dh = a.heads, a.dim_head
        if self.C != 512 or self.dh != 64 or self.heads * self.dh != self.C:
            raise NotImplementedError("omnitok_b200 kernels are specialised for embedding_dim=512, heads x dim_head = 8 x 64")
        self.p, self.pt, self.cin = a.patch_size, a.temporal_patch_size, a.image_channels
        self.ws = a.twod_window_size
        self.causal_attn = bool(a.causal_in_temporal_transformer)
        self.causal_peg = bool(a.causal_in_peg)
        self.rope = a.spatial_pos == "rope"
        self.use_vae = bool(model.use_vae)
        self.cd = a.codebook_dim
        self.l2 = bool(a.l2_code)
        if not self.use_vae and self.cd != 8:
            raise NotImplementedError(f"--codebook_dim {self.cd}: the VQ search / post_vq kernels are specialised for "
                                      "codebook_dim 8 (every shipped config); VAE mode takes 8 latent channels as well")
        self.planes = self.math == _cabi.MATH_F16X3
        self.attn_f16 = self.planes and os.environ.get("OMT_ATTN_F16", "1") == "1"
        self.static_u = self.planes and os.environ.get("OMT_STATIC_U", "1") == "1"
        if a.attn_dropout != 0 or a.ff_dropout != 0:
            raise NotImplementedError("non-zero dropout reaches SDPA even in eval in the reference (attention.py:451); rejected")
        self._ws: Dict[Tuple, Workspace] = {}
        self._tables: Dict[Tuple, torch.Tensor] = {}
        sd = {k: v for k, v in model.state_dict().items()}
        self._pack(sd, a)

    def _pack(self, sd, a):
        dev, m = self.device, self.math
        f32 = lambda t: t.detach().to(device=dev, dtype=torch.float32).contiguous()
        self.inner = sd["encoder.enc_spatial_transformer.layers.0.3.4.weight"].shape[1]
        self.ku = L.round_up(self.inner, 64 if self.planes else 32)

        def PL(weight, bias, **kw):
            return PackedLinear(weight, bias, dev, m, **kw)

        def lin(name, bias=True, **kw):
            return PL(sd[name + ".weight"], sd.get(name + ".bias") if bias else None, **kw)

        def t_layer(lp):
            d = {"kind": "t"}
            d["peg_w"] = f32(sd[lp + ".0.dsconv.weight"].reshape(self.C, 27).t())
            d["peg_b"] = f32(sd[lp + ".0.dsconv.bias"])
            ap = lp + ".1"
            d["norm_g"], d["norm_b"] = f32(sd[ap + ".norm.gamma"]), f32(sd[ap + ".norm.beta"])
            d["q_scale"], d["k_scale"] = f32(sd[ap + ".q_scale"]), f32(sd[ap + ".k_scale"])
            d["q_ps"], d["k_ps"] = L.pow2_scale(float(d["q_scale"].abs().max())), L.pow2_scale(float(d["k_scale"].abs().max()))
            d["to_qkv"] = PL(torch.cat([sd[ap + ".to_q.weight"], sd[ap + ".to_kv.weight"]], dim=0), None, row_scaled=True)
            d["to_out"] = lin(ap + ".to_out", bias=False)
            ff(d, lp + ".3")
            return d

        def w_layer(lp):
            d = {"kind": "w"}
            ap = lp + ".1"
            d["norm_g"], d["norm_b"] = f32(sd[ap + ".norm.gamma"]), f32(sd[ap + ".norm.beta"])
            d["bias"] = L.window_bias(sd[ap + ".relative_position_bias_table"].detach().float().cpu(),
                                      sd[ap + ".relative_position_index"].cpu(), self.ws).to(dev)
            d["qkv"] = lin(ap + ".qkv", bias=False, row_scaled=True)
            d["proj"] = lin(ap + ".proj")
            ff(d, lp + ".3")
            return d

        def ff(d, fp):
            d["ff_g"], d["ff_b"] = f32(sd[fp + ".0.weight"]), f32(sd[fp + ".0.bias"])
            d["ff1"] = PL(sd[fp + ".1.weight"], None, geglu=(self.inner, self.ku), row_scaled=True)
            w1 = sd[fp + ".1.weight"].detach().float()
            ln_bound = float(d["ff_g"].abs().max()) * math.sqrt(self.C) + float(d["ff_b"].norm())
            u_bound = (ln_bound * float(w1[:self.inner].norm(dim=1).max())) * (ln_bound * float(w1[self.inner:].norm(dim=1).max()))
            d["u_scale"] = L.pow2_scale(u_bound) if self.static_u else 0.0
            d["ff2"] = PL(sd[fp + ".4.weight"], None, k_pad=self.ku, row_scaled=self.static_u)

        def transformer(pre, block):
            layers = []
            for i, blk in enumerate(block):
                if blk == "t":
                    layers.append(t_layer(f"{pre}.layers.{i}"))
                elif blk == "w":
                    layers.append(w_layer(f"{pre}.layers.{i}"))
                else:
                    raise NotImplementedError(f"block type {blk!r}: pooling/upsampling blocks are outside the shipped configs")
            return {"layers": layers, "out_g": f32(sd[pre + ".norm_out.gamma"]), "out_b": f32(sd[pre + ".norm_out.beta"])}

        tb = "t" * a.temporal_depth
        self.enc_spatial = transformer("encoder.enc_spatial_transformer", a.enc_block)
        self.enc_temporal = transformer("encoder.enc_temporal_transformer", tb)
        self.dec_temporal = transformer("decoder.dec_temporal_transformer", tb)
        self.dec_spatial = transformer("decoder.dec_spatial_transformer", a.dec_block)

        self.has_window = "w" in (a.enc_block + a.dec_block)
        self.pe = {}
        self.cnn = getattr(a, "patch_embed", "linear") == "cnn"
        if self.cnn:
            def bn_affine(pre):
                g, b = sd[pre + ".weight"].float(), sd[pre + ".bias"].float()
                rm, rv = sd[pre + ".running_mean"].float(), sd[pre + ".running_var"].float()
                s_ = g / torch.sqrt(rv + 1e-5)
                return s_, b - rm * s_
            for key, pre in (("first", "encoder.to_patch_emb_first_frame"), ("rest", "encoder.to_patch_emb")):
                w = sd[pre + ".0.weight"].float().reshape(self.C, -1)
                s_, t_ = bn_affine(pre + ".1")
                self.pe[key] = dict(ln1_g=None, ln1_b=None, ln2_g=None, ln2_b=None,
                                    lin=PL(w * s_[:, None], sd[pre + ".0.bias"].float() * s_ + t_, row_scaled=True))
            self.px = {}
            for key, pre in (("first", "decoder.to_pixels_first_frame"), ("rest", "decoder.to_pixels")):
                wt = sd[pre + ".1.weight"].float()
                per_c = wt[0, 0].numel()
                s_, t_ = bn_affine(pre + ".2")
                w = wt.reshape(self.C, -1).t() * s_.repeat_interleave(per_c)[:, None]
                bias = (sd[pre + ".1.bias"].float() * s_ + t_).repeat_interleave(per_c)
                self.px[key] = PL(w.contiguous(), bias, row_scaled=True)
        else:
            for key, pre in (("first", "encoder.to_patch_emb_first_frame"), ("rest", "encoder.to_patch_emb")):
                self.pe[key] = dict(ln1_g=f32(sd[pre + ".1.weight"]), ln1_b=f32(sd[pre + ".1.bias"]), lin=lin(pre + ".2", row_scaled=True),
                                    ln2_g=f32(sd[pre + ".3.weight"]), ln2_b=f32(sd[pre + ".3.bias"]))
            self.px = {"first": lin("decoder.to_pixels_first_frame.0", row_scaled=True),
                       "rest": lin("decoder.to_pixels.0", row_scaled=True)}
        self.pre_w, self.pre_b = f32(sd["pre_vq_conv.1.weight"]), f32(sd["pre_vq_conv.1.bias"])
        self.post_w, self.post_b = f32(sd["post_vq_conv.1.weight"]), f32(sd["post_vq_conv.1.bias"])
        E = sd["codebook.embeddings"].detach().float().cpu()
        self.n_codes = E.shape[0]
        self.n_codes_padded = L.round_up(self.n_codes, 64)
        if not self.use_vae and self.n_codes_padded > VQ_MAX_CODES:
            raise NotImplementedError(f"--n_codes {self.n_codes}: the VQ search kernel holds an eighth of the codebook in "
                                      f"shared memory and takes at most {VQ_MAX_CODES} codes")
        e2 = (E.t() ** 2).sum(dim=0)
        pad = self.n_codes_padded - self.n_codes
        self.E = torch.cat([E, E.new_zeros(pad, E.shape[1])]).to(dev).contiguous()
        self.e2 = torch.cat([e2, e2.new_full((pad,), math.inf)]).to(dev).contiguous()

    @staticmethod
    def fuse_qkprep(M: int) -> bool:
        return os.environ.get("OMT_FUSE_QKPREP", "1") != "0"

    def _workspace(self, M: int) -> Workspace:
        ws = self._ws.get(M)
        if ws is None:
            kmax = self.cin * self.pt * self.p * self.p
            ws = Workspace(self.device, M, self.C, self.ku, kmax, max(self.cd, 16), self.planes)
            if ws.counts.numel() < self.n_codes:
                ws.counts = torch.zeros(self.n_codes, device=self.device, dtype=torch.int32)
            while len(self._ws) >= 3:
                self._ws.pop(next(iter(self._ws)))
            self._ws[M] = ws
        return ws

    def _table(self, key, fn):
        t = self._tables.get(key)
        if t is None:
            t = fn()
            t = tuple(x.to(self.device) for x in t) if isinstance(t, tuple) else t.to(self.device)
            self._tables[key] = t
        return t

    def _linear(self, A, lda, lin: PackedLinear, C, ldc, M, *, a_map=(0, 0, 0), c_map=(0, 0, 0), residual=None,
                ldr=0, epi=_cabi.EPI_NONE, bias=True):
        _cabi.call("omt_linear", A, lda, a_map[0], a_map[1], a_map[2], lin.w, lin.w_lo, C, ldc, c_map[0], c_map[1],
                   c_map[2], M, lin.n, lin.k, lin.bias if bias else None, residual, ldr, epi, lin.math)

    def _linear_h(self, A: Planes, lin: PackedLinear, M, *, C=None, ldc=0, U: Optional[Planes] = None, A2: Optional[Planes] = None,
                  n_split=0, a_map=(0, 0, 0), c_map=(0, 0, 0), residual=None, ldr=0, epi=_cabi.EPI_NONE, qk=None,
                  planes=None, a_uniform=0.0, u_scale=0.0):
        if ((A.rs is not None) or a_uniform > 0.0) != lin.row_scaled:
            raise RuntimeError("operand planes and weight planes are in different f16x3 forms (row-scaled vs 2^11-scaled lo)")
        kw = dict(a_hi=A.hi, a_lo=A.lo, lda=A.ld, a_seg=a_map[0], a_seg_stride=a_map[1], a_seg_off=a_map[2],
                  w_hi=lin.w, w_lo=lin.w_lo, c=C, ldc=ldc, c_seg=c_map[0], c_seg_stride=c_map[1], c_seg_off=c_map[2],
                  M=M, N=lin.n, K=lin.k, bias=lin.bias, residual=residual, ldr=ldr, epilogue=epi)
        if A.rs is not None:
            kw.update(a_rs=A.rs, w_scale=lin.w_scale)
        elif a_uniform > 0.0:
            kw.update(a_rs_uniform=a_uniform, w_scale=lin.w_scale)
        if u_scale > 0.0:
            kw.update(u_scale=u_scale)
        if A2 is not None:
            kw.update(a2_hi=A2.hi, a2_lo=A2.lo, a2_rs=A2.rs, n_split=n_split)
        if U is not None:
            kw.update(u_hi=U.hi, u_lo=U.lo, ldu=U.ld)
        if qk is not None:
            kw.update(q_scale=qk[0], k_scale=qk[1], rope_cos=qk[2], rope_sin=qk[3], qk_cols=qk[4], tokens=qk[5])
        if planes is not None:
            kw.update(q_plane_scale=planes[0], k_plane_scale=planes[1], vinv=planes[2])
        _cabi.linear_h(**kw)

    def _ln(self, x, y, g, b, M, C=None, seg=(0, 0, 0)):
        C = C or self.C
        _cabi.call("omt_layernorm", x, C, y, C, g, b, M, C, 1e-5, seg[0], seg[1], seg[2])

    def _ln_h(self, x, yp: Planes, g, b, M, xp: Optional[Planes] = None):
        C = self.C
        _cabi.call("omt_layernorm_h", x, C, None, 0, yp.hi, yp.lo, yp.rs, None if xp is None else xp.hi,
                   None if xp is None else xp.lo, None if xp is None else xp.rs, yp.ld, g, b, M, C, 1e-5, 0, 0, 0)

    def _transformer(self, tr, ws: Workspace, B, T, h, w, temporal: bool, out_planes: Optional[Planes] = None):
        C, N, M = self.C, h * w, ws.M
        H = self.planes
        q_ptr = ws.QKV.data_ptr()
        k_ptr, v_ptr = q_ptr + C * 4, q_ptr + 2 * C * 4
        ld3 = 3 * C
        o, o_hi, o_lo = (None, ws.Op.hi, ws.Op.lo) if H else (ws.O, None, None)
        for lyr in tr["layers"]:
            if lyr["kind"] == "t":
                _cabi.call("omt_peg_volume", ws.X, ws.Y, lyr["peg_w"], lyr["peg_b"], B, T, h, w, C, int(temporal),
                           int(self.causal_peg))
                ws.X, ws.Y = ws.Y, ws.X
                wq = lyr["to_qkv"]
                cos = sin = None
                if (not temporal) and self.rope:
                    cos, sin = self._table(("rope", N), lambda: L.rope_tables(N, self.dh))
                f16_core = H and self.attn_f16 and (not temporal) and N % 128 == 0
                if f16_core:
                    self._ln_h(ws.X, ws.XNp, lyr["norm_g"], lyr["norm_b"], M, xp=ws.XSp)
                    self._linear_h(ws.XNp, wq, M, U=ws.QKVp, A2=ws.XSp, n_split=C, epi=_cabi.EPI_QKV_PLANES,
                                   qk=(lyr["q_scale"], lyr["k_scale"], cos, sin, 2 * C, N),
                                   planes=(lyr["q_ps"], lyr["k_ps"], ws.vinv))
                elif H:
                    self._ln_h(ws.X, ws.XNp, lyr["norm_g"], lyr["norm_b"], M, xp=ws.XSp)
                    self._linear_h(ws.XNp, wq, M, C=q_ptr, ldc=ld3, A2=ws.XSp, n_split=C, epi=_cabi.EPI_QKV,
                                   qk=(lyr["q_scale"], lyr["k_scale"], cos, sin, 2 * C, N))
                else:
                    self._ln(ws.X, ws.XN, lyr["norm_g"], lyr["norm_b"], M)
                    if self.fuse_qkprep(M):
                        _cabi.call("omt_linear2", ws.XN, ws.X, C, C, wq.w, wq.w_lo, q_ptr, ld3, M, wq.n, wq.k, wq.math,
                                   lyr["q_scale"], lyr["k_scale"], cos, sin, 2 * C, N)
                    else:
                        _cabi.call("omt_linear2", ws.XN, ws.X, C, C, wq.w, wq.w_lo, q_ptr, ld3, M, wq.n, wq.k, wq.math,
                                   None, None, None, None, 0, 0)
                        _cabi.call("omt_qk_prep", q_ptr, ld3, k_ptr, ld3, lyr["q_scale"], lyr["k_scale"], cos, sin, M, N,
                                   self.heads)
                if f16_core:
                    ph, pl = ws.QKVp.hi.data_ptr(), ws.QKVp.lo.data_ptr()
                    _cabi.call("omt_attn_spatial_h", ph, pl, ld3, ph + 2 * C, pl + 2 * C, ld3, ph + 4 * C, pl + 4 * C, ld3,
                               ws.vinv, lyr["q_ps"] * lyr["k_ps"], None, o_hi, o_lo, C, B * T, N, self.heads, 8.0)
                elif temporal:
                    _cabi.call("omt_attn_temporal", q_ptr, ld3, k_ptr, ld3, v_ptr, ld3, o, o_hi, o_lo, C, B, T, N,
                               self.heads, 8.0, int(self.causal_attn))
                else:
                    _cabi.call("omt_attn_spatial", q_ptr, ld3, k_ptr, ld3, v_ptr, ld3, o, o_hi, o_lo, C, B * T, N,
                               self.heads, 8.0)
                proj = lyr["to_out"]
            else:
                if H:
                    self._ln_h(ws.X, ws.XNp, lyr["norm_g"], lyr["norm_b"], M)
                    self._linear_h(ws.XNp, lyr["qkv"], M, C=q_ptr, ldc=ld3)
                else:
                    self._ln(ws.X, ws.XN, lyr["norm_g"], lyr["norm_b"], M)
                    self._linear(ws.XN, C, lyr["qkv"], q_ptr, ld3, M)
                _cabi.call("omt_attn_window", q_ptr, ld3, k_ptr, ld3, v_ptr, ld3, o, o_hi, o_lo, C, lyr["bias"], B * T, h,
                           w, self.ws, self.heads, float(self.dh) ** -0.5)
                proj = lyr["proj"]
            if H:
                self._linear_h(ws.Op, proj, M, C=ws.X, ldc=C, residual=ws.X, ldr=C)
                self._ln_h(ws.X, ws.XNp, lyr["ff_g"], lyr["ff_b"], M)
                us = lyr["u_scale"]
                self._linear_h(ws.XNp, lyr["ff1"], M, U=ws.Up, epi=_cabi.EPI_GEGLU, u_scale=us)
                self._linear_h(ws.Up, lyr["ff2"], M, C=ws.X, ldc=C, residual=ws.X, ldr=C, a_uniform=(1.0 / us if us > 0 else 0.0))
            else:
                self._linear(ws.O, C, proj, ws.X, C, M, residual=ws.X, ldr=C)
                self._ln(ws.X, ws.XN, lyr["ff_g"], lyr["ff_b"], M)
                self._linear(ws.XN, C, lyr["ff1"], ws.U, self.ku, M, epi=_cabi.EPI_GEGLU)
                self._linear(ws.U, self.ku, lyr["ff2"], ws.X, C, M, residual=ws.X, ldr=C)
        if out_planes is not None:
            self._ln_h(ws.X, out_planes, tr["out_g"], tr["out_b"], M)
        else:
            self._ln(ws.X, ws.X, tr["out_g"], tr["out_b"], M)

    def _shape(self, shape):
        B, Cin, T, H, W = shape
        if Cin != self.cin:
            raise ValueError(f"expected {self.cin} channels, got {Cin}")
        assert (T - 1) % self.pt == 0, (f"number of frames ({T}) minus one ({T - 1}) must be divisible by temporal "
                                        f"patch size ({self.pt})")
        if H != W or H % self.p != 0:
            raise ValueError(f"frames must be square with side a multiple of the patch size {self.p} (got {H}x{W})")
        if self.has_window and (self.ws * self.ws != 64 or (H // self.p) % self.ws != 0):
            raise ValueError(f"window blocks need twod_window_size 8 and a token grid divisible by it (got window "
                             f"{self.ws}, grid {H // self.p}x{W // self.p}): omt_attn_window is specialised for 8x8 windows")
        if ((H // self.p) * (W // self.p)) % 64 != 0:
            raise ValueError(f"tokens per frame ({(H // self.p) * (W // self.p)}) must be a multiple of 64 (attention tiles)")
        return B, T, H, W, 1 + (T - 1) // self.pt, H // self.p, W // self.p

    @staticmethod
    def graphs_enabled() -> bool:
        return os.environ.get("OMT_CUDA_GRAPH", "1") != "0"

    def _run(self, ws: Workspace, key, body):
        if not self.graphs_enabled():
            return body()
        g = ws.graphs.get(key)
        if g is None:
            body()
            ws.graphs[key] = "warm"
        elif g == "warm":
            graph = torch.cuda.CUDAGraph()
            torch.cuda.synchronize(self.device)
            n0 = _cabi.launch_count
            with torch.cuda.graph(graph):
                body()
            ws.graphs[key] = (graph, _cabi.launch_count - n0)
            graph.replay()
        else:
            g[0].replay()
            _cabi.launch_count += g[1]

    def _encode_body(self, ws: Workspace, gather, dims, mode: str):
        B, T, H, W, Tp, h, w = dims
        N, C = h * w, self.C
        ws.reset()
        k1 = self.cin * self.p * self.p

        def embed(pe, first, rows, K, cmap):
            if self.planes:
                Pp = Planes.__new__(Planes)
                Pp.hi, Pp.lo, Pp.ld, Pp.rs = ws.Pp.hi, ws.Pp.lo, K, ws.Pp.rs
                gather(first, None, Pp.hi, Pp.lo, Pp.rs, pe["ln1_g"], pe["ln1_b"])
                self._linear_h(Pp, pe["lin"], rows, C=ws.X, ldc=C, c_map=cmap)
            else:
                gather(first, ws.P, None, None, None, pe["ln1_g"], pe["ln1_b"])
                self._linear(ws.P, K, pe["lin"], ws.X, C, rows, c_map=cmap)
            if not self.cnn:
                self._ln(ws.X, ws.X, pe["ln2_g"], pe["ln2_b"], rows, seg=cmap)

        embed(self.pe["first"], 1, B * N, k1, (N, Tp * N, 0))
        if Tp > 1:
            embed(self.pe["rest"], 0, B * (Tp - 1) * N, k1 * self.pt, ((Tp - 1) * N, Tp * N, N))
        self._transformer(self.enc_spatial, ws, B, Tp, h, w, temporal=False)
        self._transformer(self.enc_temporal, ws, B, Tp, h, w, temporal=True)
        cd = self.pre_w.shape[0]
        z = ws.z.view(-1)[: ws.M * cd].view(ws.M, cd)
        if mode == "vq":
            ws.counts.zero_()
            _cabi.call("omt_vq_fused", ws.X, C, self.pre_w, self.pre_b, C, int(self.l2), z, self.E, self.e2, ws.M,
                       self.n_codes_padded, ws.idx, ws.counts)
        else:
            _cabi.call("omt_pre_vq", ws.X, C, self.pre_w, self.pre_b, z, ws.M, C, cd, 0)

    def encode(self, x: torch.Tensor, mode: str):
        dims = self._shape(tuple(x.shape))
        B, T, H, W, Tp, h, w = dims
        ws = self._workspace(B * Tp * h * w)
        if ws.x_in is None or ws.x_in.shape != x.shape:
            ws.x_in = torch.empty_like(x, memory_format=torch.contiguous_format)
            ws.graphs = {k: v for k, v in ws.graphs.items() if not k[0].startswith("enc")}
        ws.x_in.copy_(x)

        def gather(first, *out):
            _cabi.call("omt_patchify_ln", ws.x_in, *out, B, self.cin, T, H, W, self.p, self.pt, first, 1e-5)

        self._run(ws, ("enc:" + mode, tuple(x.shape)), lambda: self._encode_body(ws, gather, dims, mode))
        return ws, (B, Tp, h, w)

    def encode_u8(self, frames: torch.Tensor, mode: str, norm: L.U8Norm):
        if frames.dtype != torch.uint8 or frames.ndim != 5:
            raise TypeError(f"encode_u8 takes (B, T, H, W, C) uint8 frames, got {tuple(frames.shape)} {frames.dtype}")
        Bf, Tf, Hf, Wf, Cf = frames.shape
        dims = self._shape((Bf, Cf, Tf, Hf, Wf))
        B, T, H, W, Tp, h, w = dims
        ws = self._workspace(B * Tp * h * w)
        if ws.u8_in is None or ws.u8_in.shape != frames.shape:
            ws.u8_in = torch.empty(frames.shape, device=self.device, dtype=torch.uint8)
            ws.u8_sel = torch.empty(B, device=self.device, dtype=torch.int32)
            ws.graphs = {k: v for k, v in ws.graphs.items() if not k[0].startswith("enc_u8")}
        ws.u8_in.copy_(frames)
        lut = self._table(("u8norm", norm), lambda: L.u8_norm_table(norm, self.cin))
        sel = ws.u8_sel if norm.max_test else None

        def gather(first, *out):
            _cabi.call("omt_patchify_ln_u8", ws.u8_in, lut, sel, *out, B, self.cin, T, H, W, self.p, self.pt, first, 1e-5)

        def body():
            if sel is not None:
                _cabi.call("omt_u8_norm_select", ws.u8_in, B, T * H * W * self.cin, sel)
            self._encode_body(ws, gather, dims, mode)

        self._run(ws, ("enc_u8:" + mode, tuple(frames.shape), norm), body)
        return ws, (B, Tp, h, w)

    def z_view(self, ws: Workspace) -> torch.Tensor:
        return self._dense(ws.z, ws.M, self.pre_w.shape[0])

    @staticmethod
    def _dense(buf: torch.Tensor, M: int, cols: int) -> torch.Tensor:
        return buf.view(-1)[: M * cols].view(M, cols)

    def zq_view(self, ws: Workspace) -> torch.Tensor:
        return self._dense(ws.zq, ws.M, self.post_w.shape[1])

    def _decode_body(self, ws: Workspace, dims, mode: str, u8=None):
        B, Tp, h, w = dims
        N, M, C = h * w, ws.M, self.C
        ws.reset()
        cdp = self.post_w.shape[1]
        if mode == "idx":
            _cabi.call("omt_post_vq", ws.idx_in, self.E, None, None, None, self.post_w, self.post_b, ws.X, M, C, cdp)
        elif mode == "idx_st":
            _cabi.call("omt_post_vq", ws.idx_in, self.E, None, self.z_view(ws), self.zq_view(ws), self.post_w,
                       self.post_b, ws.X, M, C, cdp)
        else:
            _cabi.call("omt_post_vq", None, None, self._dense(ws.zc_in, M, cdp), None, None, self.post_w, self.post_b,
                       ws.X, M, C, cdp)
        self._transformer(self.dec_temporal, ws, B, Tp, h, w, temporal=True)
        self._transformer(self.dec_spatial, ws, B, Tp, h, w, temporal=False, out_planes=ws.XNp if self.planes else None)
        T = 1 + (Tp - 1) * self.pt
        H, W = h * self.p, w * self.p
        k1 = self.cin * self.p * self.p

        def pixels(px, first, rows, K, amap):
            if self.planes:
                self._linear_h(ws.XNp, px, rows, C=ws.P, ldc=K, a_map=amap)
            else:
                self._linear(ws.X, C, px, ws.P, K, rows, a_map=amap)
            if u8 is None:
                _cabi.call("omt_unpatchify", ws.P, ws.video, B, self.cin, T, H, W, self.p, self.pt, first)
            else:
                _cabi.call("omt_unpatchify_u8", ws.P, ws.video_u8, B, self.cin, T, H, W, self.p, self.pt, first, *u8)

        pixels(self.px["first"], 1, B * N, k1, (N, Tp * N, 0))
        if Tp > 1:
            pixels(self.px["rest"], 0, B * (Tp - 1) * N, k1 * self.pt, ((Tp - 1) * N, Tp * N, N))

    def decode(self, dims, *, idx=None, zc=None, straight_through=False, u8=None) -> torch.Tensor:
        B, Tp, h, w = dims
        ws = self._workspace(B * Tp * h * w)
        vshape = (B, self.cin, 1 + (Tp - 1) * self.pt, h * self.p, w * self.p)
        if ws.video is None or tuple(ws.video.shape) != vshape:
            ws.video = torch.empty(vshape, device=self.device, dtype=torch.float32)
            ws.video_u8 = torch.empty((B, vshape[2], vshape[3], vshape[4], self.cin), device=self.device, dtype=torch.uint8)
            ws.graphs = {k: v for k, v in ws.graphs.items() if not k[0].startswith("dec")}
        if idx is not None:
            ws.idx_in.copy_(idx.reshape(-1))
            mode = "idx_st" if straight_through else "idx"
        else:
            self._dense(ws.zc_in, ws.M, zc.shape[1]).copy_(zc)
            mode = "zc"
        u8 = None if u8 is None else tuple(float(v) for v in u8)
        self._run(ws, ("dec:" + mode, dims, u8), lambda: self._decode_body(ws, dims, mode, u8))
        return ws.video.clone() if u8 is None else ws.video_u8.clone()
```

Before: 3617.

## Emit per-row-scaled f16 output planes from attention for to_out projection

Attention kernels (f16 spatial and temporal) can now write their output hi/lo f16 planes with a per-row scale and a row-scale vector. The to_out projection then runs in row-scaled mode, which is meant to preserve split-f16 accuracy and may allow a cheaper GEMM path. The spatial kernel gains a producer warp that computes the V max across heads, with extra mbarriers to hand it over. The GEMM residual epilogue is also restructured so residual loads are hoisted. In exchange this adds synchronization and a per-item reduction over vinv, and the temporal path now requires heads == 8.

```diff
diff --git a/include/omnitok_b200.h b/include/omnitok_b200.h
--- a/include/omnitok_b200.h
+++ b/include/omnitok_b200.h
@@ -80,6 +80,11 @@
                        float* o, uint16_t* o_hi, uint16_t* o_lo, int ldo, int n_seq, int N, int heads, float scale,
                        omt_stream_t stream);
 
+int omt_attn_spatial_h_rs(const uint16_t* q_hi, const uint16_t* q_lo, int ldq, const uint16_t* k_hi, const uint16_t* k_lo,
+                          int ldk, const uint16_t* v_hi, const uint16_t* v_lo, int ldv, const float* vinv, float qk_plane_scale,
+                          float* o, uint16_t* o_hi, uint16_t* o_lo, float* o_rs, int ldo, int n_seq, int N, int heads,
+                          float scale, omt_stream_t stream);
+
 int omt_attn_window(const float* q, int ldq, const float* k, int ldk, const float* v, int ldv,
                     float* o, uint16_t* o_hi, uint16_t* o_lo, int ldo, const float* bias, int n_frames, int h, int w, int ws, int heads,
                     float scale, omt_stream_t stream);
@@ -87,6 +92,9 @@
 int omt_attn_temporal(const float* q, int ldq, const float* k, int ldk, const float* v, int ldv,
                       float* o, uint16_t* o_hi, uint16_t* o_lo, int ldo, int B, int T, int N, int heads, float scale, int causal,
                       omt_stream_t stream);
+int omt_attn_temporal_rs(const float* q, int ldq, const float* k, int ldk, const float* v, int ldv,
+                         float* o, uint16_t* o_hi, uint16_t* o_lo, float* o_rs, int ldo, int B, int T, int N, int heads,
+                         float scale, int causal, omt_stream_t stream);
 
 int omt_pre_vq(const float* x, int ldx, const float* Wt, const float* b, float* z, int M, int C, int cd,
                int l2, omt_stream_t stream);
diff --git a/omnitokenizer_b200/_cabi.py b/omnitokenizer_b200/_cabi.py
--- a/omnitokenizer_b200/_cabi.py
+++ b/omnitokenizer_b200/_cabi.py
@@ -61,6 +61,10 @@
                                 c_void_p, c_int, c_int, c_int, c_int, c_int, c_float, c_void_p]),
     "omt_attn_temporal": (c_int, [c_void_p, c_int, c_void_p, c_int, c_void_p, c_int, c_void_p, c_void_p, c_void_p, c_int,
                                   c_int, c_int, c_int, c_int, c_float, c_int, c_void_p]),
+    "omt_attn_spatial_h_rs": (c_int, [c_void_p, c_void_p, c_int, c_void_p, c_void_p, c_int, c_void_p, c_void_p, c_int, c_void_p,
+                                      c_float, c_void_p, c_void_p, c_void_p, c_void_p, c_int, c_int, c_int, c_int, c_float, c_void_p]),
+    "omt_attn_temporal_rs": (c_int, [c_void_p, c_int, c_void_p, c_int, c_void_p, c_int, c_void_p, c_void_p, c_void_p, c_void_p,
+                                     c_int, c_int, c_int, c_int, c_int, c_float, c_int, c_void_p]),
     "omt_pre_vq": (c_int, [c_void_p, c_int, c_void_p, c_void_p, c_void_p, c_int, c_int, c_int, c_int, c_void_p]),
     "omt_vq_search": (c_int, [c_void_p, c_void_p, c_void_p, c_int, c_int, c_void_p, c_void_p, c_void_p]),
     "omt_vq_fused": (c_int, [c_void_p, c_int, c_void_p, c_void_p, c_int, c_int, c_void_p, c_void_p, c_void_p, c_int, c_int,
diff --git a/omnitokenizer_b200/csrc/attention_f16.cu b/omnitokenizer_b200/csrc/attention_f16.cu
--- a/omnitokenizer_b200/csrc/attention_f16.cu
+++ b/omnitokenizer_b200/csrc/attention_f16.cu
@@ -23,6 +23,7 @@
   const float* vinv;
   long long rows;
   float* o; uint16_t* o_hi; uint16_t* o_lo; int ldo;
+  float* o_rs;
   int N, heads, items;
   float scale_log2;
 };
@@ -38,7 +39,9 @@
   uint64_t& q_empty = bars[1];
   uint64_t* full = bars + 2;
   uint64_t* empty = full + STAGES;
-  float* vmax = reinterpret_cast<float*>(bars + 2 + 2 * STAGES);
+  uint64_t* vall_full = empty + STAGES;
+  uint64_t* vall_empty = vall_full + 2;
+  float* vmax = reinterpret_cast<float*>(bars + 2 + 2 * STAGES + 4);
 
   const int tid = threadIdx.x, warp = tid >> 5, lane = tid & 31;
   const int ntiles = a.N / KT, nqt = a.N / QT;
@@ -48,6 +51,7 @@
     mbar_init(&q_full, 1);
     mbar_init(&q_empty, 256);
     for (int s = 0; s < STAGES; ++s) { mbar_init(&full[s], 1); mbar_init(&empty[s], 2); }
+    for (int b = 0; b < 2; ++b) { mbar_init(&vall_full[b], 1); mbar_init(&vall_empty[b], 256); }
     fence_barrier_init();
   }
   __syncthreads();
@@ -99,6 +103,26 @@
           }
         }
       }
+    } else if (warp == 1 && a.o_rs != nullptr) {
+      uint32_t c = 0;
+      for (int item = blockIdx.x; item < a.items; item += gridDim.x, ++c) {
+        int row_q0, row_k0, col0, head;
+        decode(item, row_q0, row_k0, col0, head);
+        float vall = 0.f;
+        for (int i = 4 * lane; i < a.N; i += 128)
+#pragma unroll 4
+          for (int h = 0; h < a.heads; ++h) {
+            const float4 v = __ldg(reinterpret_cast<const float4*>(a.vinv + (size_t)h * a.rows + row_k0 + i));
+            vall = fmaxf(vall, fmaxf(fmaxf(v.x, v.y), fmaxf(v.z, v.w)));
+          }
+        vall = warp_max(vall);
+        const int b = c & 1;
+        mbar_wait(&vall_empty[b], ((c >> 1) & 1) ^ 1);
+        if (lane == 0) {
+          vmax[2 + b] = vall;
+          mbar_arrive(&vall_full[b]);
+        }
+      }
     }
   } else {
     setmaxnreg_inc<CONSUMER_REGS>();
@@ -117,7 +141,7 @@
       decode(item, row_q0, row_k0, col0, head);
       mbar_wait(&q_full, c & 1);
       float p_scale, p_inv;
-      row_scale(*vmax, p_scale, p_inv);
+      row_scale(vmax[0], p_scale, p_inv);
       uint32_t qh[16], ql[16];
 #pragma unroll
       for (int kk = 0; kk < 4; ++kk)
@@ -239,13 +263,27 @@
       step(p_b, p_a, j + 1, false);
       it += ntiles;
 
+      float o_scale = 1.f, o_inv = 1.f;
+      if (a.o_rs != nullptr) {
+        mbar_wait(&vall_full[c & 1], (c >> 1) & 1);
+        row_scale(32768.f * vmax[2 + (c & 1)], o_scale, o_inv);
+        mbar_arrive(&vall_empty[c & 1]);
+      }
 #pragma unroll
       for (int h = 0; h < 2; ++h) {
         float l = l_run[h];
         l += __shfl_xor_sync(0xffffffffu, l, 1);
         l += __shfl_xor_sync(0xffffffffu, l, 2);
         const float inv = p_inv / l;
-        const size_t ooff = (size_t)(row_q0 + wg * 64 + rl0 + 8 * h) * a.ldo + col0 + 2 * qd;
+        const int row = row_q0 + wg * 64 + rl0 + 8 * h;
+        const size_t ooff = (size_t)row * a.ldo + col0 + 2 * qd;
+        if (a.o_rs != nullptr) {
+#pragma unroll
+          for (int jj = 0; jj < 8; ++jj)
+            store_split2u_s(a.o_hi, a.o_lo, ooff + 8 * jj, make_float2(o_acc[4 * jj + 2 * h] * inv, o_acc[4 * jj + 2 * h + 1] * inv), o_scale);
+          if (head == 0 && qd == 0) a.o_rs[row] = o_inv;
+          continue;
+        }
 #pragma unroll
         for (int jj = 0; jj < 8; ++jj) {
           const float2 ov = make_float2(o_acc[4 * jj + 2 * h] * inv, o_acc[4 * jj + 2 * h + 1] * inv);
@@ -287,10 +325,10 @@
 
 using namespace omt;
 
-extern "C" int omt_attn_spatial_h(const uint16_t* q_hi, const uint16_t* q_lo, int ldq, const uint16_t* k_hi,
-                                  const uint16_t* k_lo, int ldk, const uint16_t* v_hi, const uint16_t* v_lo, int ldv,
-                                  const float* vinv, float qk_plane_scale, float* o, uint16_t* o_hi, uint16_t* o_lo, int ldo,
-                                  int n_seq, int N, int heads, float scale, omt_stream_t stream) {
+extern "C" int omt_attn_spatial_h_rs(const uint16_t* q_hi, const uint16_t* q_lo, int ldq, const uint16_t* k_hi,
+                                     const uint16_t* k_lo, int ldk, const uint16_t* v_hi, const uint16_t* v_lo, int ldv,
+                                     const float* vinv, float qk_plane_scale, float* o, uint16_t* o_hi, uint16_t* o_lo,
+                                     float* o_rs, int ldo, int n_seq, int N, int heads, float scale, omt_stream_t stream) {
   using namespace af16;
   OMT_ENTER();
   OMT_REQUIRE(q_hi && q_lo && k_hi && k_lo && v_hi && v_lo && vinv && (o || o_hi) && ((o_hi == nullptr) == (o_lo == nullptr)),
@@ -300,6 +338,7 @@
   OMT_REQUIRE(((uintptr_t)q_hi | (uintptr_t)q_lo | (uintptr_t)k_hi | (uintptr_t)k_lo | (uintptr_t)v_hi | (uintptr_t)v_lo | (uintptr_t)vinv |
                (uintptr_t)o | (uintptr_t)o_hi | (uintptr_t)o_lo) % 16 == 0, "omt_attn_spatial_h: pointers must be 16-byte aligned");
   OMT_REQUIRE(heads > 0 && heads <= 65535 && n_seq <= 65535 && qk_plane_scale > 0.f, "omt_attn_spatial_h: bad arguments");
+  OMT_REQUIRE(o_rs == nullptr || o_hi != nullptr, "omt_attn_spatial_h: o_rs needs the output planes");
   if (n_seq == 0) return OMT_OK;
   const long long rows = (long long)n_seq * N;
   const long long items = rows / QT * heads;
@@ -324,9 +363,17 @@
     OMT_REQUIRE(per_sm > 0, "omt_attn_spatial_h: no CTA fits on an SM of device %d", dev);
     resident[dev] = per_sm * sms;
   }
-  Args a{vinv, rows, o, o_hi, o_lo, ldo, N, heads, (int)items, scale * 1.4426950408889634f / qk_plane_scale};
+  Args a{vinv, rows, o, o_hi, o_lo, ldo, o_rs, N, heads, (int)items, scale * 1.4426950408889634f / qk_plane_scale};
   const dim3 grid(items < resident[dev] ? (int)items : resident[dev]);
   OMT_CUDA(launch_k(attn_f16_kernel, grid, dim3(THREADS), SMEM, (cudaStream_t)stream, tmQh, tmQl, tmKh, tmKl, tmVh, tmVl, a));
   OMT_LAUNCH_CHECK();
   return OMT_OK;
 }
+
+extern "C" int omt_attn_spatial_h(const uint16_t* q_hi, const uint16_t* q_lo, int ldq, const uint16_t* k_hi,
+                                  const uint16_t* k_lo, int ldk, const uint16_t* v_hi, const uint16_t* v_lo, int ldv,
+                                  const float* vinv, float qk_plane_scale, float* o, uint16_t* o_hi, uint16_t* o_lo, int ldo,
+                                  int n_seq, int N, int heads, float scale, omt_stream_t stream) {
+  return omt_attn_spatial_h_rs(q_hi, q_lo, ldq, k_hi, k_lo, ldk, v_hi, v_lo, ldv, vinv, qk_plane_scale, o, o_hi, o_lo, nullptr, ldo,
+                               n_seq, N, heads, scale, stream);
+}
diff --git a/omnitokenizer_b200/csrc/attention_fp32.cu b/omnitokenizer_b200/csrc/attention_fp32.cu
--- a/omnitokenizer_b200/csrc/attention_fp32.cu
+++ b/omnitokenizer_b200/csrc/attention_fp32.cu
@@ -164,13 +164,14 @@
   }
 }
 
-template <int T>
+template <int T, bool RS>
 __global__ void __launch_bounds__(256) attn_temporal_kernel(const float* __restrict__ q, int ldq,
                                                             const float* __restrict__ k, int ldk,
                                                             const float* __restrict__ v, int ldv,
                                                             float* __restrict__ o, uint16_t* __restrict__ o_hi,
-                                                            uint16_t* __restrict__ o_lo, int ldo, int B,
-                                                            int N, int heads, float scale, int causal) {
+                                                            uint16_t* __restrict__ o_lo, float* __restrict__ o_rs, int ldo,
+                                                            int B, int N, int heads, float scale, int causal) {
+  __shared__ __align__(16) float rmax[RS ? T : 1][8];
   pdl_sync();
   const int lane = threadIdx.x & 31;
   const long long wid = (long long)blockIdx.x * (blockDim.x >> 5) + (threadIdx.x >> 5);
@@ -182,6 +183,7 @@
   const int b = (int)(bn / N);
   const size_t col = (size_t)head * 64 + 2 * lane;
   float2 kr[T], vr[T], qr[T];
+  float2 ro[T];
 #pragma unroll
   for (int t = 0; t < T; ++t) {
     const size_t row = ((size_t)b * T + t) * N + n;
@@ -217,18 +219,42 @@
       }
     }
     const float2 ov = make_float2(ox / den, oy / den);
-    if (o_hi != nullptr) store_split2(o_hi, o_lo, row * ldo + col, ov);
-    else *reinterpret_cast<float2*>(o + row * ldo + col) = ov;
+    if constexpr (RS) {
+      ro[i] = ov;
+      const float m = warp_max(fmaxf(fabsf(ov.x), fabsf(ov.y)));
+      if (lane == 0) rmax[i][head] = m;
+    } else if (o_hi != nullptr) {
+      store_split2(o_hi, o_lo, row * ldo + col, ov);
+    } else {
+      *reinterpret_cast<float2*>(o + row * ldo + col) = ov;
+    }
+  }
+  if constexpr (RS) {
+    __syncthreads();
+#pragma unroll
+    for (int i = 0; i < T; ++i) {
+      const size_t row = ((size_t)b * T + i) * N + n;
+      float s, inv;
+      row_scale(fmaxf(max4abs(*reinterpret_cast<const float4*>(&rmax[i][0])), max4abs(*reinterpret_cast<const float4*>(&rmax[i][4]))),
+                s, inv);
+      store_split2u_s(o_hi, o_lo, row * ldo + col, ro[i], s);
+      if (head == 0 && lane == 0) o_rs[row] = inv;
+    }
   }
 }
 
 template <int T>
 static int launch_temporal(const float* q, int ldq, const float* k, int ldk, const float* v, int ldv,
-                           float* o, uint16_t* o_hi, uint16_t* o_lo, int ldo, int B, int N, int heads, float scale, int causal,
-                           cudaStream_t st) {
+                           float* o, uint16_t* o_hi, uint16_t* o_lo, float* o_rs, int ldo, int B, int N, int heads, float scale,
+                           int causal, cudaStream_t st) {
   const long long warps = (long long)B * N * heads;
   const unsigned blocks = (unsigned)((warps + 7) / 8);
-  OMT_CUDA(launch_k(attn_temporal_kernel<T>, dim3(blocks), dim3(256), 0, st, q, ldq, k, ldk, v, ldv, o, o_hi, o_lo, ldo, B, N, heads, scale, causal));
+  if (o_rs != nullptr)
+    OMT_CUDA(launch_k(attn_temporal_kernel<T, true>, dim3(blocks), dim3(256), 0, st, q, ldq, k, ldk, v, ldv, o, o_hi, o_lo, o_rs, ldo,
+                      B, N, heads, scale, causal));
+  else
+    OMT_CUDA(launch_k(attn_temporal_kernel<T, false>, dim3(blocks), dim3(256), 0, st, q, ldq, k, ldk, v, ldv, o, o_hi, o_lo, o_rs, ldo,
+                      B, N, heads, scale, causal));
   OMT_LAUNCH_CHECK();
   return OMT_OK;
 }
@@ -303,16 +329,18 @@
   return OMT_OK;
 }
 
-extern "C" int omt_attn_temporal(const float* q, int ldq, const float* k, int ldk, const float* v, int ldv,
-                                 float* o, uint16_t* o_hi, uint16_t* o_lo, int ldo, int B, int T, int N, int heads,
-                                 float scale, int causal, omt_stream_t stream) {
+extern "C" int omt_attn_temporal_rs(const float* q, int ldq, const float* k, int ldk, const float* v, int ldv,
+                                    float* o, uint16_t* o_hi, uint16_t* o_lo, float* o_rs, int ldo, int B, int T, int N, int heads,
+                                    float scale, int causal, omt_stream_t stream) {
   OMT_ENTER();
   int rc = check_attn_ptrs("omt_attn_temporal", q, ldq, k, ldk, v, ldv, o, o_hi, o_lo, ldo);
   if (rc) return rc;
   OMT_REQUIRE(T >= 1 && T <= 17, "omt_attn_temporal: T'=%d unsupported (1..17)", T);
+  OMT_REQUIRE(o_rs == nullptr || (o_hi != nullptr && heads == 8),
+              "omt_attn_temporal: o_rs needs the output planes and heads == 8 (a CTA holds the whole row)");
   if ((long long)B * N == 0) return OMT_OK;
   cudaStream_t st = (cudaStream_t)stream;
-#define OMT_T_CASE(t) case t: return launch_temporal<t>(q, ldq, k, ldk, v, ldv, o, o_hi, o_lo, ldo, B, N, heads, scale, causal, st);
+#define OMT_T_CASE(t) case t: return launch_temporal<t>(q, ldq, k, ldk, v, ldv, o, o_hi, o_lo, o_rs, ldo, B, N, heads, scale, causal, st);
   switch (T) {
     OMT_T_CASE(1) OMT_T_CASE(2) OMT_T_CASE(3) OMT_T_CASE(4) OMT_T_CASE(5) OMT_T_CASE(6) OMT_T_CASE(7)
     OMT_T_CASE(8) OMT_T_CASE(9) OMT_T_CASE(10) OMT_T_CASE(11) OMT_T_CASE(12) OMT_T_CASE(13) OMT_T_CASE(14)
@@ -321,3 +349,9 @@
 #undef OMT_T_CASE
   return OMT_E_ARG;
 }
+
+extern "C" int omt_attn_temporal(const float* q, int ldq, const float* k, int ldk, const float* v, int ldv,
+                                 float* o, uint16_t* o_hi, uint16_t* o_lo, int ldo, int B, int T, int N, int heads,
+                                 float scale, int causal, omt_stream_t stream) {
+  return omt_attn_temporal_rs(q, ldq, k, ldk, v, ldv, o, o_hi, o_lo, nullptr, ldo, B, T, N, heads, scale, causal, stream);
+}
diff --git a/omnitokenizer_b200/csrc/gemm_wgmma.cuh b/omnitokenizer_b200/csrc/gemm_wgmma.cuh
--- a/omnitokenizer_b200/csrc/gemm_wgmma.cuh
+++ b/omnitokenizer_b200/csrc/gemm_wgmma.cuh
@@ -155,25 +155,49 @@
       }
     }
   } else {
-#pragma unroll
-    for (int h = 0; h < 2; ++h) {
-      const int m = mrow[h];
-      if (m < g.M) {
-        const long long prow = map_row(m, g.c_seg, g.c_seg_stride, g.c_seg_off);
-#pragma unroll
-        for (int j = 0; j < BN / 8; ++j) {
-          const int n = n0 + 8 * j + 2 * qd;
-          if (n < g.N) {
-            float2 o = make_float2(v[h][2 * j], v[h][2 * j + 1]);
-            if (g.bias != nullptr) {
-              const float2 bb = __ldg(reinterpret_cast<const float2*>(g.bias + n));
-              o.x += bb.x; o.y += bb.y;
+    long long prow[2];
+#pragma unroll
+    for (int h = 0; h < 2; ++h) prow[h] = map_row(mrow[h] < g.M ? mrow[h] : 0, g.c_seg, g.c_seg_stride, g.c_seg_off);
+    if (g.residual == nullptr) {
+#pragma unroll
+      for (int h = 0; h < 2; ++h) {
+        if (mrow[h] < g.M) {
+#pragma unroll
+          for (int j = 0; j < BN / 8; ++j) {
+            const int n = n0 + 8 * j + 2 * qd;
+            if (n < g.N) {
+              float2 o = make_float2(v[h][2 * j], v[h][2 * j + 1]);
+              if (g.bias != nullptr) {
+                const float2 bb = __ldg(reinterpret_cast<const float2*>(g.bias + n));
+                o.x += bb.x; o.y += bb.y;
+              }
+              *reinterpret_cast<float2*>(g.c + prow[h] * g.ldc + n) = o;
             }
-            if (g.residual != nullptr) {
-              const float2 r = *reinterpret_cast<const float2*>(g.residual + prow * g.ldr + n);
-              o.x += r.x; o.y += r.y;
+          }
+        }
+      }
+    } else {
+#pragma unroll
+      for (int h = 0; h < 2; ++h) {
+        if (mrow[h] < g.M) {
+          float2 r[BN / 8];
+#pragma unroll
+          for (int j = 0; j < BN / 8; ++j) {
+            const int n = n0 + 8 * j + 2 * qd;
+            if (n < g.N) r[j] = *reinterpret_cast<const float2*>(g.residual + prow[h] * g.ldr + n);
+          }
+#pragma unroll
+          for (int j = 0; j < BN / 8; ++j) {
+            const int n = n0 + 8 * j + 2 * qd;
+            if (n < g.N) {
+              float2 o = make_float2(v[h][2 * j], v[h][2 * j + 1]);
+              if (g.bias != nullptr) {
+                const float2 bb = __ldg(reinterpret_cast<const float2*>(g.bias + n));
+                o.x += bb.x; o.y += bb.y;
+              }
+              o.x += r[j].x; o.y += r[j].y;
+              *reinterpret_cast<float2*>(g.c + prow[h] * g.ldc + n) = o;
             }
-            *reinterpret_cast<float2*>(g.c + prow * g.ldc + n) = o;
           }
         }
       }
diff --git a/omnitokenizer_b200/csrc/omt_common.cuh b/omnitokenizer_b200/csrc/omt_common.cuh
--- a/omnitokenizer_b200/csrc/omt_common.cuh
+++ b/omnitokenizer_b200/csrc/omt_common.cuh
@@ -106,6 +106,12 @@
   const float2 h = unpack_f16x2(hi2);
   lo2 = pack_f16x2_sat(a - h.x, b - h.y);
 }
+__device__ __forceinline__ void store_split2u_s(uint16_t* hi, uint16_t* lo, size_t off, float2 v, float scale) {
+  uint32_t h, l;
+  split2u(v.x * scale, v.y * scale, h, l);
+  *reinterpret_cast<uint32_t*>(hi + off) = h;
+  *reinterpret_cast<uint32_t*>(lo + off) = l;
+}
 __device__ __forceinline__ void store_split4u(uint16_t* hi, uint16_t* lo, size_t off, float4 v, float scale) {
   uint2 h, l;
   split2u(v.x * scale, v.y * scale, h.x, l.x);
diff --git a/omnitokenizer_b200/engine.py b/omnitokenizer_b200/engine.py
--- a/omnitokenizer_b200/engine.py
+++ b/omnitokenizer_b200/engine.py
@@ -1,5 +1,6 @@
 from __future__ import annotations
 
+import copy
 import math
 import os
 from typing import Dict, Optional, Tuple
@@ -54,7 +55,7 @@
 
 
 class Workspace:
-    def __init__(self, device, M: int, C: int, ku: int, kmax: int, cd: int, planes: bool):
+    def __init__(self, device, M: int, C: int, ku: int, kmax: int, cd: int, planes: bool, o_rowscale: bool = False):
         f = dict(device=device, dtype=torch.float32)
         self.M = M
         self.buf0 = torch.empty(M, C, **f)
@@ -64,7 +65,10 @@
         self.P = torch.empty(M, kmax, **f)
         if planes:
             self.XNp, self.XSp = Planes(device, M, C, True), Planes(device, M, C, True)
-            self.Op, self.Up = Planes(device, M, C), Planes(device, M, ku)
+            self.Up = Planes(device, M, ku)
+            self.Op = Planes(device, M, C, o_rowscale)
+            self.Op_e = copy.copy(self.Op)
+            self.Op_e.rs = None
             self.Pp = Planes(device, M, kmax, True)
             self.QKVp = Planes(device, M, 3 * C)
             self.vinv = torch.empty(C // 64, M, device=device, dtype=torch.float32)
@@ -120,6 +124,7 @@
         self.planes = self.math == _cabi.MATH_F16X3
         self.attn_f16 = self.planes and os.environ.get("OMT_ATTN_F16", "1") == "1"
         self.static_u = self.planes and os.environ.get("OMT_STATIC_U", "1") == "1"
+        self.o_rowscale = self.planes and os.environ.get("OMT_O_ROWSCALE", "1") == "1"
         if a.attn_dropout != 0 or a.ff_dropout != 0:
             raise NotImplementedError("non-zero dropout reaches SDPA even in eval in the reference (attention.py:451); rejected")
         self._ws: Dict[Tuple, Workspace] = {}
@@ -139,7 +144,7 @@
         def lin(name, bias=True, **kw):
             return PL(sd[name + ".weight"], sd.get(name + ".bias") if bias else None, **kw)
 
-        def t_layer(lp):
+        def t_layer(lp, spatial):
             d = {"kind": "t"}
             d["peg_w"] = f32(sd[lp + ".0.dsconv.weight"].reshape(self.C, 27).t())
             d["peg_b"] = f32(sd[lp + ".0.dsconv.bias"])
@@ -148,7 +153,9 @@
             d["q_scale"], d["k_scale"] = f32(sd[ap + ".q_scale"]), f32(sd[ap + ".k_scale"])
             d["q_ps"], d["k_ps"] = L.pow2_scale(float(d["q_scale"].abs().max())), L.pow2_scale(float(d["k_scale"].abs().max()))
             d["to_qkv"] = PL(torch.cat([sd[ap + ".to_q.weight"], sd[ap + ".to_kv.weight"]], dim=0), None, row_scaled=True)
-            d["to_out"] = lin(ap + ".to_out", bias=False)
+            d["to_out"] = lin(ap + ".to_out", bias=False, row_scaled=self.o_rowscale)
+            if spatial and self.o_rowscale:
+                d["to_out_e"] = lin(ap + ".to_out", bias=False)
             ff(d, lp + ".3")
             return d
 
@@ -172,11 +179,11 @@
             d["u_scale"] = L.pow2_scale(u_bound) if self.static_u else 0.0
             d["ff2"] = PL(sd[fp + ".4.weight"], None, k_pad=self.ku, row_scaled=self.static_u)
 
-        def transformer(pre, block):
+        def transformer(pre, block, spatial=True):
             layers = []
             for i, blk in enumerate(block):
                 if blk == "t":
-                    layers.append(t_layer(f"{pre}.layers.{i}"))
+                    layers.append(t_layer(f"{pre}.layers.{i}", spatial))
                 elif blk == "w":
                     layers.append(w_layer(f"{pre}.layers.{i}"))
                 else:
@@ -185,8 +192,8 @@
 
         tb = "t" * a.temporal_depth
         self.enc_spatial = transformer("encoder.enc_spatial_transformer", a.enc_block)
-        self.enc_temporal = transformer("encoder.enc_temporal_transformer", tb)
-        self.dec_temporal = transformer("decoder.dec_temporal_transformer", tb)
+        self.enc_temporal = transformer("encoder.enc_temporal_transformer", tb, spatial=False)
+        self.dec_temporal = transformer("decoder.dec_temporal_transformer", tb, spatial=False)
         self.dec_spatial = transformer("decoder.dec_spatial_transformer", a.dec_block)
 
         self.has_window = "w" in (a.enc_block + a.dec_block)
@@ -238,7 +245,7 @@
         ws = self._ws.get(M)
         if ws is None:
             kmax = self.cin * self.pt * self.p * self.p
-            ws = Workspace(self.device, M, self.C, self.ku, kmax, max(self.cd, 16), self.planes)
+            ws = Workspace(self.device, M, self.C, self.ku, kmax, max(self.cd, 16), self.planes, self.o_rowscale)
             if ws.counts.numel() < self.n_codes:
                 ws.counts = torch.zeros(self.n_codes, device=self.device, dtype=torch.int32)
             while len(self._ws) >= 3:
@@ -299,7 +306,9 @@
         k_ptr, v_ptr = q_ptr + C * 4, q_ptr + 2 * C * 4
         ld3 = 3 * C
         o, o_hi, o_lo = (None, ws.Op.hi, ws.Op.lo) if H else (ws.O, None, None)
+        o_rs = ws.Op.rs if H else None
         for lyr in tr["layers"]:
+            op = ws.Op if H else None
             if lyr["kind"] == "t":
                 _cabi.call("omt_peg_volume", ws.X, ws.Y, lyr["peg_w"], lyr["peg_b"], B, T, h, w, C, int(temporal),
                            int(self.causal_peg))
@@ -330,15 +339,18 @@
                                    self.heads)
                 if f16_core:
                     ph, pl = ws.QKVp.hi.data_ptr(), ws.QKVp.lo.data_ptr()
-                    _cabi.call("omt_attn_spatial_h", ph, pl, ld3, ph + 2 * C, pl + 2 * C, ld3, ph + 4 * C, pl + 4 * C, ld3,
-                               ws.vinv, lyr["q_ps"] * lyr["k_ps"], None, o_hi, o_lo, C, B * T, N, self.heads, 8.0)
+                    _cabi.call("omt_attn_spatial_h_rs", ph, pl, ld3, ph + 2 * C, pl + 2 * C, ld3, ph + 4 * C, pl + 4 * C, ld3,
+                               ws.vinv, lyr["q_ps"] * lyr["k_ps"], None, o_hi, o_lo, o_rs, C, B * T, N, self.heads, 8.0)
+                    proj = lyr["to_out"]
                 elif temporal:
-                    _cabi.call("omt_attn_temporal", q_ptr, ld3, k_ptr, ld3, v_ptr, ld3, o, o_hi, o_lo, C, B, T, N,
+                    _cabi.call("omt_attn_temporal_rs", q_ptr, ld3, k_ptr, ld3, v_ptr, ld3, o, o_hi, o_lo, o_rs, C, B, T, N,
                                self.heads, 8.0, int(self.causal_attn))
+                    proj = lyr["to_out"]
                 else:
                     _cabi.call("omt_attn_spatial", q_ptr, ld3, k_ptr, ld3, v_ptr, ld3, o, o_hi, o_lo, C, B * T, N,
                                self.heads, 8.0)
-                proj = lyr["to_out"]
+                    proj = lyr.get("to_out_e", lyr["to_out"])
+                    op = ws.Op_e if H else None
             else:
                 if H:
                     self._ln_h(ws.X, ws.XNp, lyr["norm_g"], lyr["norm_b"], M)
@@ -349,8 +361,9 @@
                 _cabi.call("omt_attn_window", q_ptr, ld3, k_ptr, ld3, v_ptr, ld3, o, o_hi, o_lo, C, lyr["bias"], B * T, h,
                            w, self.ws, self.heads, float(self.dh) ** -0.5)
                 proj = lyr["proj"]
+                op = ws.Op_e if H else None
             if H:
-                self._linear_h(ws.Op, proj, M, C=ws.X, ldc=C, residual=ws.X, ldr=C)
+                self._linear_h(op, proj, M, C=ws.X, ldc=C, residual=ws.X, ldr=C)
                 self._ln_h(ws.X, ws.XNp, lyr["ff_g"], lyr["ff_b"], M)
                 us = lyr["u_scale"]
                 self._linear_h(ws.XNp, lyr["ff1"], M, U=ws.Up, epi=_cabi.EPI_GEGLU, u_scale=us)
```

Result: faster. 3815 (median of 6 runs) (+5.5%).
